# xXCoffeeColaXc/WeatherConverter

Measured on NVIDIA B200. Metric: guided translation images/sec (256x512, T steps) at 1/2/4/8 B200 vs host CPU, higher is better.
Workload: dtype bf16

## Files before the change

include/wc_b200.h:

```cpp
#ifndef WC_B200_H_
#define WC_B200_H_

#include <stddef.h>
#include <stdint.h>

#ifdef __cplusplus
extern "C" {
#endif

typedef uint16_t wc_bf16;

const char* wc_last_error(void);
int wc_abi_version(void);
long long wc_launch_count(void);

void wc_profile_begin(void);
int wc_profile_end(double* ms_by_class, long long* count_by_class, double* work_by_class);
int wc_profile_detail(int cap, int* cls, double* ms, double* work, int* info);

int wc_ddpm_step(const float* xt, const float* eps, const float* z, float* out, float* mean_out, float* sigz_out,
                 size_t n_per_sample, int batch, float beta, float sqrt_one_minus_acp, float sqrt_alpha, float sigma,
                 void* stream);
int wc_ddpm_step_batched(const float* xt, const float* eps, const float* z, float* out, float* mean_out,
                         float* sigz_out, size_t n_per_sample, int batch, const float* betas, const float* alphas,
                         const float* sqrt_one_minus_acp, const int64_t* t, int num_timesteps, void* stream);
int wc_ddpm_step_indexed(const float* xt, const float* eps, const float* z, float* out, float* mean_out, float* sigz_out,
                         size_t n_per_sample, int batch, const float* coef_tables, const int64_t* t_dev, int num_timesteps,
                         void* stream);
int wc_ddim_step(const float* xt, const float* eps, const float* z, float* out, float* mean_out, float* sigz_out,
                 size_t n_per_sample, int batch, float a_t, float s_t, float a_prev, float d, float sigma, void* stream);
int wc_ddim_step_indexed(const float* xt, const float* eps, const float* z, float* out, float* mean_out, float* sigz_out,
                         size_t n_per_sample, int batch, const float* coef_tables, const int64_t* t_dev, int num_timesteps,
                         void* stream);
int wc_add_noise(const float* x0, const float* noise, float* out, size_t n_per_sample, int batch,
                 const float* sqrt_acp, const float* sqrt_one_minus_acp, const int64_t* t, int num_timesteps, void* stream);

int wc_set_time_factor_table(const float* factor_host, int half);
int wc_time_embedding(const int64_t* t, int n, int dim, float* out, void* stream);

int wc_sgg_update(const float* grad, const float* mu, const float* sigz, float* out, float* mag_out, int batch, int h,
                  int w, int pool, float lambda, void* stream);

int wc_lcg_prepare(const float* sr_xt, const int64_t* gt, float* x_masked, int64_t* gt_masked, int batch, int num_classes,
                   int H, int W, void* stream);
int wc_lcg_combine(const float* pooled_grads, const int64_t* gt, const float* mu, const float* sigz, float* out, int batch,
                   int num_classes, int h, int w, int pool, float lambda, void* stream);

size_t wc_groupnorm_workspace_bytes(int batch);
int wc_groupnorm_silu(const wc_bf16* x, wc_bf16* y, int batch, int hw, int channels, int ldx, int ldy,
                      const float* gamma, const float* beta, float eps, int silu, void* workspace, void* stream);
int wc_conv2d(const wc_bf16* x, int batch, int H, int W, int Cin, int ldx, const float* weight, const float* bias,
              int Cout, int K, int stride, int pad, int dil, int transposed, const float* rowbias,
              const wc_bf16* residual, int ldr, const wc_bf16* x2, int Cin2, int ldx2, const float* weight2, int relu,
              wc_bf16* y, int ldy, void* stream);
int wc_conv_in(const float* x, const float* weight, const float* bias, const float* scale, const float* shift,
               wc_bf16* y, int batch, int H, int W, int Cout, int K, int stride, int pad, int ldy, int relu,
               void* stream);
int wc_conv_out(const wc_bf16* x, const float* weight, const float* bias, float* y, int batch, int H, int W, int Cin,
                int K, int ldx, int tanh_out, void* stream);
int wc_conv2d_dgrad(const wc_bf16* dz, int batch, int Ho, int Wo, int Cout, const float* weight, int Cin, int K, int stride,
                    int dil, const wc_bf16* residual, const wc_bf16* mask, wc_bf16* dx, void* stream);
int wc_maxpool3x3s2(const wc_bf16* x, wc_bf16* y, uint8_t* idx, int batch, int H, int W, int C, void* stream);
int wc_maxpool3x3s2_bwd(const wc_bf16* dy, const uint8_t* idx, const wc_bf16* x, wc_bf16* dx, int batch, int H, int W, int C,
                        void* stream);
int wc_bilinear(const wc_bf16* x, wc_bf16* y, int batch, int Hi, int Wi, int Ho, int Wo, int C, void* stream);
int wc_bilinear_bwd(const wc_bf16* dy, const wc_bf16* mask, wc_bf16* dx, int batch, int Hi, int Wi, int Ho, int Wo, int C,
                    void* stream);
int wc_seg_loss_head(const float* logits_lo, const int64_t* labels, int* n_valid_ws, int64_t* pred, float* dlogit_hi,
                     float* loss, float* logits_hi, wc_bf16* dlogit_lo, int batch, int h, int w, int H, int W, void* stream);
int wc_conv1_dgrad(const wc_bf16* dz, const float* weight, const float* scale, float* dx, int batch, int H, int W, void* stream);
int wc_nchw_f32_to_nhwc_bf16(const float* x, wc_bf16* y, int batch, int C, int hw, int ldy, void* stream);
int wc_nhwc_bf16_to_nchw_f32(const wc_bf16* x, float* y, int batch, int C, int hw, int ldx, void* stream);
int wc_attention(const wc_bf16* q, const wc_bf16* k, const wc_bf16* vt, wc_bf16* out, int batch, int heads, int ntok,
                 int hd, int ldo, void* stream);
int wc_attention_scaled(const wc_bf16* q, const wc_bf16* k, const wc_bf16* vt, wc_bf16* out, int batch, int heads, int ntok,
                        int hd, int ldo, float scale, void* stream);

int wc_ddpm_grid_u8(const float* x, uint8_t* out, int batch, int H, int W, int nrow, int padding, void* stream);
int wc_postprocess_u8(const float* x, uint8_t* out, int batch, int H, int W, const float* mean3_host, const float* std3_host, void* stream);
int wc_label_encode(const uint8_t* label_ids, int Ws, const int* ytab, const int* xtab, int top, int left, int Hc, int Wc,
                    const int64_t* lut, int nlut, int64_t* out, void* stream);
int wc_resample_u8(const uint8_t* in, uint8_t* tmp, uint8_t* out, int Hin, int Win, int Hout, int Wout, int channels, const int* bounds_h,
                   const int* kk_h, int ksize_h, const int* bounds_v, const int* kk_v, int ksize_v, void* stream);
int wc_u8_to_tensor(const uint8_t* in, int Win, int top, int left, int Hc, int Wc, int mode, const float* mean3_host, const float* std3_host,
                    float* out, void* stream);

int wc_attention_lse(const wc_bf16* q, const wc_bf16* k, const wc_bf16* vt, wc_bf16* out, float* lse, int batch, int heads,
                     int ntok, int hd, int ldo, void* stream);
int wc_attention_bwd(const wc_bf16* q, const wc_bf16* k, const wc_bf16* v, const wc_bf16* o, const wc_bf16* d_o, const float* lse,
                     float* d_scratch, wc_bf16* dqkv, int batch, int heads, int ntok, int hd, void* stream);
int wc_conv2d_wgrad(const wc_bf16* x, const wc_bf16* dy, int batch, int H, int W, int Cin, int Cout, int K, int stride, int pad,
                    int dil, int transposed, const wc_bf16* x2, int Cin2, float* dw, float* dw2, void* stream);
size_t wc_groupnorm_bwd_workspace_bytes(int batch, int channels);
int wc_groupnorm_silu_bwd(const wc_bf16* x, const wc_bf16* dy, wc_bf16* dx, int batch, int hw, int channels, const float* gamma,
                          const float* beta, float eps, int silu, const void* fwd_workspace, const wc_bf16* add1,
                          const wc_bf16* add2, float* dgamma, float* dbeta, void* workspace, void* stream);
int wc_colsum(const wc_bf16* x, int batch, int hw, int channels, float* out_rows, float* out_total, void* workspace, void* stream);
int wc_mse_loss_grad(const float* pred, const float* target, float* dpred, size_t n, float grad_scale, float* loss, void* scratch,
                     void* stream);
size_t wc_boundary_wgrad_scratch_bytes(void);
int wc_boundary_wgrad(const wc_bf16* wide, const float* narrow, int batch, int H, int W, int sign, float* dw, float* dbias,
                      void* scratch, void* stream);
int wc_adam_step(float* p, const float* g, float* m, float* v, size_t n, float lr, float beta1, float beta2, float eps, int step,
                 float grad_scale, void* stream);

typedef struct wc_unet wc_unet;
typedef struct {
  int im_channels, im_size, time_emb_dim, num_down_layers, num_mid_layers, num_up_layers, num_heads;
  int n_down_channels;
  int down_channels[8];
  int n_mid_channels;
  int mid_channels[8];
  int down_sample[8];
  int n_attn_resolutions;
  int attn_resolutions[8];
} wc_unet_config;
int wc_unet_create(wc_unet** out, const wc_unet_config* cfg, int n_params, const char* const* names,
                   const float* const* ptrs, const int64_t* numels, void* stream);
void wc_unet_destroy(wc_unet* net);
size_t wc_unet_workspace_bytes(const wc_unet* net, int batch, int H, int W);
int wc_unet_forward(wc_unet* net, const float* x, const int64_t* t, int n_t, float* out, int batch, int H, int W,
                    void* workspace, size_t workspace_bytes, void* stream);
double wc_unet_flops(const wc_unet* net);
int wc_unet_launches(const wc_unet* net);

typedef struct wc_unet_train wc_unet_train;
int wc_unet_train_create(wc_unet_train** out, const wc_unet_config* cfg, int n_params, const char* const* names,
                         float* const* params, float* const* grads);
void wc_unet_train_destroy(wc_unet_train* net);
size_t wc_unet_train_workspace_bytes(wc_unet_train* net, int batch, int H, int W);
int wc_unet_train_bind(wc_unet_train* net, int batch, int H, int W, void* workspace, size_t workspace_bytes, void* stream);
int wc_unet_train_forward(wc_unet_train* net, const float* x, const int64_t* t, const float* target, float* pred_out,
                          float* loss_out, float grad_scale, int repack, void* stream);
int wc_unet_train_num_backward_ops(const wc_unet_train* net);
int wc_unet_train_backward(wc_unet_train* net, int op_begin, int op_end, void* stream);
int wc_unet_train_backward_seeded(wc_unet_train* net, const float* dpred, float* dx, int param_grads, void* stream);
int wc_unet_train_grad_ready_op(const wc_unet_train* net, const char* name);
double wc_unet_train_flops(const wc_unet_train* net, int backward);

typedef struct wc_legacy_unet wc_legacy_unet;
int wc_legacy_unet_create(wc_legacy_unet** out, int n_params, const char* const* names, const float* const* ptrs,
                          const int64_t* numels);
void wc_legacy_unet_destroy(wc_legacy_unet* net);
size_t wc_legacy_unet_workspace_bytes(wc_legacy_unet* net, int batch, int size);
int wc_legacy_unet_forward(wc_legacy_unet* net, const float* x, const float* t, float* out, int batch, int size, void* workspace,
                           size_t workspace_bytes, void* stream);
double wc_legacy_unet_flops(const wc_legacy_unet* net);
int wc_legacy_unet_launches(const wc_legacy_unet* net);

typedef struct wc_seg wc_seg;
int wc_seg_create(wc_seg** out, const int* blocks_per_layer, int num_classes, int n_params, const char* const* names,
                  const float* const* ptrs, void* stream);
int wc_seg_set_output_stride(wc_seg* net, int output_stride);
void wc_seg_destroy(wc_seg* net);
size_t wc_seg_workspace_bytes(const wc_seg* net, int batch, int H, int W, int with_grad);
int wc_seg_infer(wc_seg* net, const float* x, const int64_t* labels, int64_t* pred, float* input_grad, float* loss,
                 float* logits, int batch, int H, int W, void* workspace, size_t workspace_bytes, void* stream);
int wc_seg_infer_pooled(wc_seg* net, const float* x, const int64_t* labels, int64_t* pred, float* input_grad, float* loss,
                        float* logits, int batch, int H, int W, int grad_pool, void* workspace, size_t workspace_bytes,
                        void* stream);
int wc_seg_forward(wc_seg* net, const float* x, float* logits, int batch, int H, int W, int save_for_backward, void* workspace,
                   size_t workspace_bytes, void* stream);
int wc_seg_backward_seeded(wc_seg* net, const float* dlogits, float* input_grad, void* stream);
double wc_seg_flops(const wc_seg* net, int backward);
int wc_seg_launches(const wc_seg* net);

typedef struct wc_srgan wc_srgan;
int wc_srgan_create(wc_srgan** out, int num_blocks, int upscale, int n_params, const char* const* names,
                    const float* const* ptrs, void* stream);
void wc_srgan_destroy(wc_srgan* net);
size_t wc_srgan_workspace_bytes(const wc_srgan* net, int batch, int h, int w);
int wc_srgan_forward(wc_srgan* net, const float* x, float* y, int batch, int h, int w, void* workspace,
                     size_t workspace_bytes, void* stream);
size_t wc_srgan_grad_workspace_bytes(const wc_srgan* net, int batch, int h, int w);
int wc_srgan_forward_saved(wc_srgan* net, const float* x, float* y, int batch, int h, int w, void* workspace,
                           size_t workspace_bytes, void* stream);
int wc_srgan_backward_seeded(wc_srgan* net, const float* dy, float* dx, void* stream);
double wc_srgan_flops(const wc_srgan* net);
int wc_srgan_launches(const wc_srgan* net);

#ifdef __cplusplus
}
#endif
#endif
```

weatherconverter_b200/_lib.py:

```python
import ctypes as C
import os

import torch

_HERE = os.path.dirname(os.path.abspath(__file__))
LIB_PATH = os.path.join(_HERE, "libwc_b200.so")

_lib = None

c_f32p = C.c_void_p
c_ptr = C.c_void_p


class UnetConfigStruct(C.Structure):
    _fields_ = [
        ("im_channels", C.c_int), ("im_size", C.c_int), ("time_emb_dim", C.c_int),
        ("num_down_layers", C.c_int), ("num_mid_layers", C.c_int), ("num_up_layers", C.c_int),
        ("num_heads", C.c_int),
        ("n_down_channels", C.c_int), ("down_channels", C.c_int * 8),
        ("n_mid_channels", C.c_int), ("mid_channels", C.c_int * 8),
        ("down_sample", C.c_int * 8),
        ("n_attn_resolutions", C.c_int), ("attn_resolutions", C.c_int * 8),
    ]


_SIGS = {
    "wc_last_error": (C.c_char_p, []),
    "wc_abi_version": (C.c_int, []),
    "wc_launch_count": (C.c_longlong, []),
    "wc_profile_begin": (None, []),
    "wc_profile_detail": (C.c_int, [C.c_int, C.POINTER(C.c_int), C.POINTER(C.c_double), C.POINTER(C.c_double), C.POINTER(C.c_int)]),
    "wc_profile_end": (C.c_int, [C.POINTER(C.c_double), C.POINTER(C.c_longlong), C.POINTER(C.c_double)]),
    "wc_ddpm_step": (C.c_int, [c_ptr] * 6 + [C.c_size_t, C.c_int] + [C.c_float] * 4 + [c_ptr]),
    "wc_ddpm_step_batched": (C.c_int, [c_ptr] * 6 + [C.c_size_t, C.c_int] + [c_ptr] * 4 + [C.c_int, c_ptr]),
    "wc_ddpm_step_indexed": (C.c_int, [c_ptr] * 6 + [C.c_size_t, C.c_int, c_ptr, c_ptr, C.c_int, c_ptr]),
    "wc_ddim_step": (C.c_int, [c_ptr] * 6 + [C.c_size_t, C.c_int] + [C.c_float] * 5 + [c_ptr]),
    "wc_ddim_step_indexed": (C.c_int, [c_ptr] * 6 + [C.c_size_t, C.c_int, c_ptr, c_ptr, C.c_int, c_ptr]),
    "wc_add_noise": (C.c_int, [c_ptr] * 3 + [C.c_size_t, C.c_int] + [c_ptr] * 3 + [C.c_int, c_ptr]),
    "wc_set_time_factor_table": (C.c_int, [C.POINTER(C.c_float), C.c_int]),
    "wc_time_embedding": (C.c_int, [c_ptr, C.c_int, C.c_int, c_ptr, c_ptr]),
    "wc_sgg_update": (C.c_int, [c_ptr] * 5 + [C.c_int] * 4 + [C.c_float, c_ptr]),
    "wc_lcg_prepare": (C.c_int, [c_ptr] * 4 + [C.c_int] * 4 + [c_ptr]),
    "wc_lcg_combine": (C.c_int, [c_ptr] * 5 + [C.c_int] * 5 + [C.c_float, c_ptr]),
    "wc_groupnorm_workspace_bytes": (C.c_size_t, [C.c_int]),
    "wc_groupnorm_silu": (C.c_int, [c_ptr, c_ptr] + [C.c_int] * 5 + [c_ptr, c_ptr, C.c_float, C.c_int, c_ptr, c_ptr]),
    "wc_conv2d": (C.c_int, [c_ptr] + [C.c_int] * 5 + [c_ptr, c_ptr] + [C.c_int] * 6 + [c_ptr, c_ptr, C.c_int, c_ptr,
                            C.c_int, C.c_int, c_ptr, C.c_int, c_ptr, C.c_int, c_ptr]),
    "wc_conv2d_dgrad": (C.c_int, [c_ptr] + [C.c_int] * 4 + [c_ptr] + [C.c_int] * 4 + [c_ptr] * 4),
    "wc_maxpool3x3s2": (C.c_int, [c_ptr] * 3 + [C.c_int] * 4 + [c_ptr]),
    "wc_maxpool3x3s2_bwd": (C.c_int, [c_ptr] * 4 + [C.c_int] * 4 + [c_ptr]),
    "wc_bilinear": (C.c_int, [c_ptr] * 2 + [C.c_int] * 6 + [c_ptr]),
    "wc_bilinear_bwd": (C.c_int, [c_ptr] * 3 + [C.c_int] * 6 + [c_ptr]),
    "wc_seg_loss_head": (C.c_int, [c_ptr] * 8 + [C.c_int] * 5 + [c_ptr]),
    "wc_conv1_dgrad": (C.c_int, [c_ptr] * 4 + [C.c_int] * 3 + [c_ptr]),
    "wc_conv_in": (C.c_int, [c_ptr] * 6 + [C.c_int] * 9 + [c_ptr]),
    "wc_conv_out": (C.c_int, [c_ptr] * 4 + [C.c_int] * 7 + [c_ptr]),
    "wc_nchw_f32_to_nhwc_bf16": (C.c_int, [c_ptr, c_ptr] + [C.c_int] * 4 + [c_ptr]),
    "wc_nhwc_bf16_to_nchw_f32": (C.c_int, [c_ptr, c_ptr] + [C.c_int] * 4 + [c_ptr]),
    "wc_attention": (C.c_int, [c_ptr] * 4 + [C.c_int] * 5 + [c_ptr]),
    "wc_ddpm_grid_u8": (C.c_int, [c_ptr, c_ptr] + [C.c_int] * 5 + [c_ptr]),
    "wc_postprocess_u8": (C.c_int, [c_ptr, c_ptr] + [C.c_int] * 3 + [C.POINTER(C.c_float), C.POINTER(C.c_float), c_ptr]),
    "wc_label_encode": (C.c_int, [c_ptr, C.c_int, c_ptr, c_ptr] + [C.c_int] * 4 + [c_ptr, C.c_int, c_ptr, c_ptr]),
    "wc_resample_u8": (C.c_int, [c_ptr] * 3 + [C.c_int] * 5 + [c_ptr, c_ptr, C.c_int, c_ptr, c_ptr, C.c_int, c_ptr]),
    "wc_u8_to_tensor": (C.c_int, [c_ptr] + [C.c_int] * 6 + [C.POINTER(C.c_float), C.POINTER(C.c_float), c_ptr, c_ptr]),
    "wc_attention_lse": (C.c_int, [c_ptr] * 5 + [C.c_int] * 5 + [c_ptr]),
    "wc_attention_scaled": (C.c_int, [c_ptr] * 4 + [C.c_int] * 5 + [C.c_float, c_ptr]),
    "wc_attention_bwd": (C.c_int, [c_ptr] * 8 + [C.c_int] * 4 + [c_ptr]),
    "wc_conv2d_wgrad": (C.c_int, [c_ptr, c_ptr] + [C.c_int] * 10 + [c_ptr, C.c_int, c_ptr, c_ptr, c_ptr]),
    "wc_groupnorm_bwd_workspace_bytes": (C.c_size_t, [C.c_int, C.c_int]),
    "wc_groupnorm_silu_bwd": (C.c_int, [c_ptr] * 3 + [C.c_int] * 3 + [c_ptr, c_ptr, C.c_float, C.c_int] + [c_ptr] * 7),
    "wc_colsum": (C.c_int, [c_ptr] + [C.c_int] * 3 + [c_ptr] * 4),
    "wc_mse_loss_grad": (C.c_int, [c_ptr] * 3 + [C.c_size_t, C.c_float, c_ptr, c_ptr, c_ptr]),
    "wc_boundary_wgrad_scratch_bytes": (C.c_size_t, []),
    "wc_boundary_wgrad": (C.c_int, [c_ptr, c_ptr] + [C.c_int] * 4 + [c_ptr] * 4),
    "wc_adam_step": (C.c_int, [c_ptr] * 4 + [C.c_size_t] + [C.c_float] * 4 + [C.c_int, C.c_float, c_ptr]),
    "wc_unet_create": (C.c_int, [C.POINTER(c_ptr), C.POINTER(UnetConfigStruct), C.c_int, C.POINTER(C.c_char_p),
                                 C.POINTER(c_ptr), C.POINTER(C.c_int64), c_ptr]),
    "wc_unet_destroy": (None, [c_ptr]),
    "wc_unet_workspace_bytes": (C.c_size_t, [c_ptr, C.c_int, C.c_int, C.c_int]),
    "wc_unet_forward": (C.c_int, [c_ptr, c_ptr, c_ptr, C.c_int, c_ptr, C.c_int, C.c_int, C.c_int, c_ptr, C.c_size_t,
                                  c_ptr]),
    "wc_unet_flops": (C.c_double, [c_ptr]),
    "wc_unet_launches": (C.c_int, [c_ptr]),
    "wc_unet_train_create": (C.c_int, [C.POINTER(c_ptr), C.POINTER(UnetConfigStruct), C.c_int, C.POINTER(C.c_char_p),
                                       C.POINTER(c_ptr), C.POINTER(c_ptr)]),
    "wc_unet_train_destroy": (None, [c_ptr]),
    "wc_unet_train_workspace_bytes": (C.c_size_t, [c_ptr, C.c_int, C.c_int, C.c_int]),
    "wc_unet_train_bind": (C.c_int, [c_ptr, C.c_int, C.c_int, C.c_int, c_ptr, C.c_size_t, c_ptr]),
    "wc_unet_train_forward": (C.c_int, [c_ptr] * 6 + [C.c_float, C.c_int, c_ptr]),
    "wc_unet_train_num_backward_ops": (C.c_int, [c_ptr]),
    "wc_unet_train_backward": (C.c_int, [c_ptr, C.c_int, C.c_int, c_ptr]),
    "wc_unet_train_backward_seeded": (C.c_int, [c_ptr, c_ptr, c_ptr, C.c_int, c_ptr]),
    "wc_unet_train_grad_ready_op": (C.c_int, [c_ptr, C.c_char_p]),
    "wc_unet_train_flops": (C.c_double, [c_ptr, C.c_int]),
    "wc_legacy_unet_create": (C.c_int, [C.POINTER(c_ptr), C.c_int, C.POINTER(C.c_char_p), C.POINTER(c_ptr), C.POINTER(C.c_int64)]),
    "wc_legacy_unet_destroy": (None, [c_ptr]),
    "wc_legacy_unet_workspace_bytes": (C.c_size_t, [c_ptr, C.c_int, C.c_int]),
    "wc_legacy_unet_forward": (C.c_int, [c_ptr, c_ptr, c_ptr, c_ptr, C.c_int, C.c_int, c_ptr, C.c_size_t, c_ptr]),
    "wc_legacy_unet_flops": (C.c_double, [c_ptr]),
    "wc_legacy_unet_launches": (C.c_int, [c_ptr]),
    "wc_seg_create": (C.c_int, [C.POINTER(c_ptr), C.POINTER(C.c_int), C.c_int, C.c_int, C.POINTER(C.c_char_p),
                                C.POINTER(c_ptr), c_ptr]),
    "wc_seg_set_output_stride": (C.c_int, [c_ptr, C.c_int]),
    "wc_seg_destroy": (None, [c_ptr]),
    "wc_seg_workspace_bytes": (C.c_size_t, [c_ptr, C.c_int, C.c_int, C.c_int, C.c_int]),
    "wc_seg_infer": (C.c_int, [c_ptr] * 7 + [C.c_int] * 3 + [c_ptr, C.c_size_t, c_ptr]),
    "wc_seg_infer_pooled": (C.c_int, [c_ptr] * 7 + [C.c_int] * 4 + [c_ptr, C.c_size_t, c_ptr]),
    "wc_seg_forward": (C.c_int, [c_ptr] * 3 + [C.c_int] * 4 + [c_ptr, C.c_size_t, c_ptr]),
    "wc_seg_backward_seeded": (C.c_int, [c_ptr] * 4),
    "wc_seg_flops": (C.c_double, [c_ptr, C.c_int]),
    "wc_seg_launches": (C.c_int, [c_ptr]),
    "wc_srgan_create": (C.c_int, [C.POINTER(c_ptr), C.c_int, C.c_int, C.c_int, C.POINTER(C.c_char_p), C.POINTER(c_ptr), c_ptr]),
    "wc_srgan_destroy": (None, [c_ptr]),
    "wc_srgan_workspace_bytes": (C.c_size_t, [c_ptr, C.c_int, C.c_int, C.c_int]),
    "wc_srgan_forward": (C.c_int, [c_ptr, c_ptr, c_ptr, C.c_int, C.c_int, C.c_int, c_ptr, C.c_size_t, c_ptr]),
    "wc_srgan_grad_workspace_bytes": (C.c_size_t, [c_ptr, C.c_int, C.c_int, C.c_int]),
    "wc_srgan_forward_saved": (C.c_int, [c_ptr, c_ptr, c_ptr, C.c_int, C.c_int, C.c_int, c_ptr, C.c_size_t, c_ptr]),
    "wc_srgan_backward_seeded": (C.c_int, [c_ptr] * 4),
    "wc_srgan_flops": (C.c_double, [c_ptr]),
    "wc_srgan_launches": (C.c_int, [c_ptr]),
}

EXPORTS = tuple(_SIGS.keys())


def lib():
    global _lib
    if _lib is None:
        if not os.path.exists(LIB_PATH):
            raise RuntimeError(
                f"{LIB_PATH} not found: the CUDA extension has not been built "
                "(run __graft_entry__.build()); this package has no CPU fallback")
        handle = C.CDLL(LIB_PATH)
        for name, (res, args) in _SIGS.items():
            fn = getattr(handle, name)
            fn.restype = res
            fn.argtypes = args
        _lib = handle
    return _lib


def check(rc):
    if rc != 0:
        msg = lib().wc_last_error()
        raise RuntimeError("wc_b200: " + (msg.decode() if msg else f"error {rc}"))


def require_cuda(*tensors):
    if not torch.cuda.is_available():
        raise RuntimeError("wc_b200 needs a CUDA device (sm_100a); there is no CPU fallback")
    for t in tensors:
        if t is not None and not t.is_cuda:
            raise RuntimeError("wc_b200 kernels take CUDA tensors; got a tensor on " + str(t.device))


def ptr(t):
    return None if t is None else C.c_void_p(t.data_ptr())


def stream_ptr():
    return C.c_void_p(torch.cuda.current_stream().cuda_stream)
```

weatherconverter_b200/csrc/attention.cu:

```cuda
#include "wc_host.h"
#include "wc_ptx.cuh"

#include <cstdlib>
#include <type_traits>

namespace wc {

namespace {

struct AttnArgs {
  int ntok, heads, ldo;
  float scale_log2;
  __nv_bfloat16* out;
  float* lse;
};

struct AttnMaps {
  CUtensorMap q, k, vt;
};

template <int HD, int BKV, int NQ, bool TP = false>
struct AttnCfg {
  static constexpr int kKBlocks = HD >= 64 ? HD / 64 : 1;
  static constexpr int kSwz = HD >= 64 ? 128 : HD * 2;
  static constexpr int kRowBytes = HD >= 64 ? 128 : HD * 2;
  static constexpr int kKSteps = HD >= 64 ? 4 : HD / 16;
  static constexpr uint32_t kQTile = 128 * HD * 2;
  static constexpr uint32_t kKTile = BKV * HD * 2;
  static constexpr uint32_t kVTile = HD * BKV * 2;
  static constexpr uint32_t kPTile = 128 * BKV * 2;
  static constexpr int kStages = 2;
  static constexpr uint32_t kSmem = NQ * kQTile + kStages * (kKTile + kVTile) + (TP ? 0 : NQ * kPTile) + 1024 + 256;
  static constexpr int kThreads = 128 + 128 * NQ;
  static constexpr int kColsPerQ = BKV + HD + (TP ? BKV / 2 : 0);
  static_assert(NQ * kColsPerQ <= 512, "TMEM budget");
  static constexpr uint32_t kTmemCols = NQ * kColsPerQ <= 256 ? 256 : 512;
};

template <int HD, int BKV, int NQ, int POLY, bool TP>
__global__ void __launch_bounds__(AttnCfg<HD, BKV, NQ, TP>::kThreads, 1)
attention_kernel(const __grid_constant__ AttnMaps maps, const __grid_constant__ AttnArgs p) {
  using Cfg = AttnCfg<HD, BKV, NQ, TP>;
  extern __shared__ uint8_t smem_raw[];
  const uint32_t base = (smem_u32(smem_raw) + 1023u) & ~1023u;
  const uint32_t q_smem = base;
  const uint32_t k_smem = q_smem + NQ * Cfg::kQTile;
  const uint32_t v_smem = k_smem + Cfg::kStages * Cfg::kKTile;
  const uint32_t p_smem = v_smem + Cfg::kStages * Cfg::kVTile;
  const uint32_t bars = p_smem + (TP ? 0u : NQ * Cfg::kPTile);
  const uint32_t q_full = bars;
  auto k_full = [&](int s) { return bars + 8u * (1 + s); };
  auto k_empty = [&](int s) { return bars + 8u * (3 + s); };
  auto v_full = [&](int s) { return bars + 8u * (5 + s); };
  auto v_empty = [&](int s) { return bars + 8u * (7 + s); };
  auto s_full = [&](int q) { return bars + 8u * (9 + q); };
  auto p_full = [&](int q) { return bars + 8u * (12 + q); };
  auto pv_done = [&](int q) { return bars + 8u * (15 + q); };
  const uint32_t tmem_slot = bars + 8u * 18;
  volatile uint32_t* tmem_slot_ptr = reinterpret_cast<volatile uint32_t*>(smem_raw + (tmem_slot - smem_u32(smem_raw)));

  const int warp = __shfl_sync(0xffffffffu, threadIdx.x >> 5, 0), lane = threadIdx.x & 31;
  const int bh = blockIdx.y;
  const int q0 = blockIdx.x * (128 * NQ);
  const int nkv = (p.ntok + BKV - 1) / BKV;

  if (warp == 0 && lane == 0) {
    tma_prefetch_desc(&maps.q);
    tma_prefetch_desc(&maps.k);
    tma_prefetch_desc(&maps.vt);
  }
  if (warp == 1 && lane == 0) {
    mbar_init(q_full, 1);
    for (int s = 0; s < Cfg::kStages; ++s) {
      mbar_init(k_full(s), 1); mbar_init(k_empty(s), 1);
      mbar_init(v_full(s), 1); mbar_init(v_empty(s), 1);
    }
    for (int q = 0; q < NQ; ++q) {
      mbar_init(s_full(q), 1);
      mbar_init(p_full(q), 128);
      mbar_init(pv_done(q), 1);
    }
    fence_barrier_init();
  }
  if (warp == 2) {
    tmem_alloc(tmem_slot, Cfg::kTmemCols);
    tmem_relinquish();
  }
  pdl_launch_dependents();
  pdl_wait();
  tc_fence_before();
  __syncthreads();
  tc_fence_after();
  const uint32_t tmem_base = *tmem_slot_ptr;

  if (warp == 0) {
    if (lane == 0) {
      mbar_arrive_expect_tx(q_full, NQ * Cfg::kQTile);
      for (int q = 0; q < NQ; ++q)
        for (int kb = 0; kb < Cfg::kKBlocks; ++kb)
          tma_load_3d(q_smem + q * Cfg::kQTile + kb * (128 * Cfg::kRowBytes), &maps.q, q_full, kb * 64, q0 + q * 128, bh);
      for (int j = 0; j < nkv; ++j) {
        const int s = j & 1;
        const uint32_t ph = (j >> 1) & 1u;
        mbar_wait(k_empty(s), ph ^ 1u);
        mbar_arrive_expect_tx(k_full(s), Cfg::kKTile);
        for (int kb = 0; kb < Cfg::kKBlocks; ++kb)
          tma_load_3d(k_smem + s * Cfg::kKTile + kb * (BKV * Cfg::kRowBytes), &maps.k, k_full(s), kb * 64, j * BKV, bh);
        mbar_wait(v_empty(s), ph ^ 1u);
        mbar_arrive_expect_tx(v_full(s), Cfg::kVTile);
        for (int vb = 0; vb < BKV / 64; ++vb)
          tma_load_3d(v_smem + s * Cfg::kVTile + vb * (HD * 128), &maps.vt, v_full(s), j * BKV + vb * 64, 0, bh);
      }
    }
  } else if (warp == 1) {
    {
      const uint32_t tmem_base = __shfl_sync(0xffffffffu, *tmem_slot_ptr, 0);
      const uint32_t idesc_s = umma_idesc_bf16(128, BKV);
      const uint32_t idesc_o = umma_idesc_bf16(128, HD);
      const uint64_t dq = umma_smem_desc(q_smem, Cfg::kSwz, 8 * Cfg::kRowBytes);
      const uint64_t dp = umma_smem_desc(p_smem, 128, 1024);
      const uint32_t hi_qk = umma_desc_hi(dq), hi_pv = umma_desc_hi(dp);
      const uint32_t q_lo0 = umma_desc_lo(dq), k_lo0 = q_lo0 + ((k_smem - q_smem) >> 4);
      const uint32_t p_lo0 = umma_desc_lo(dp), v_lo0 = p_lo0 - ((p_smem - v_smem) >> 4);
      auto issue_s = [&](int q, int j) {
        const uint32_t d = tmem_base + q * Cfg::kColsPerQ;
        const uint32_t q_lo = q_lo0 + q * (Cfg::kQTile >> 4), k_lo = k_lo0 + (j & 1) * (Cfg::kKTile >> 4);
#pragma unroll
        for (int kb = 0; kb < Cfg::kKBlocks; ++kb) {
#pragma unroll
          for (int k = 0; k < Cfg::kKSteps; ++k)
            umma_bf16(d, umma_desc_join(q_lo + kb * ((128 * Cfg::kRowBytes) >> 4) + 2u * k, hi_qk),
                      umma_desc_join(k_lo + kb * ((BKV * Cfg::kRowBytes) >> 4) + 2u * k, hi_qk), idesc_s, (kb | k) != 0 ? 1u : 0u);
        }
        umma_commit(s_full(q));
      };
      auto issue_pv = [&](int q, int j) {
        const uint32_t d = tmem_base + q * Cfg::kColsPerQ + BKV;
        const uint32_t p_lo = p_lo0 + q * (Cfg::kPTile >> 4), v_lo = v_lo0 + (j & 1) * (Cfg::kVTile >> 4);
#pragma unroll
        for (int vb = 0; vb < BKV / 64; ++vb) {
#pragma unroll
          for (int k = 0; k < 4; ++k)
            if (TP)
              umma_bf16_ts(d, d + HD + 8u * (vb * 4 + k), umma_desc_join(v_lo + vb * ((HD * 128) >> 4) + 2u * k, hi_pv), idesc_o,
                           (j | vb | k) != 0 ? 1u : 0u);
            else
              umma_bf16(d, umma_desc_join(p_lo + vb * ((128 * 128) >> 4) + 2u * k, hi_pv),
                        umma_desc_join(v_lo + vb * ((HD * 128) >> 4) + 2u * k, hi_pv), idesc_o, (j | vb | k) != 0 ? 1u : 0u);
        }
        umma_commit(pv_done(q));
      };
      mbar_wait(q_full, 0);
      mbar_wait(k_full(0), 0);
      tc_fence_after();
      if (elect_one_sync()) {
        for (int q = 0; q < NQ; ++q) issue_s(q, 0);
        umma_commit(k_empty(0));
      }
      __syncwarp();
      for (int j = 0; j < nkv; ++j) {
        const int s = j & 1;
        const uint32_t ph = (j >> 1) & 1u;
        mbar_wait(v_full(s), ph);
        const bool more = (j + 1 < nkv);
        if (more) mbar_wait(k_full((j + 1) & 1), ((j + 1) >> 1) & 1u);
#pragma unroll
        for (int q = 0; q < NQ; ++q) {
          mbar_wait(p_full(q), j & 1u);
          tc_fence_after();
          if (elect_one_sync()) {
            issue_pv(q, j);
            if (more) issue_s(q, j + 1);
          }
          __syncwarp();
        }
        if (elect_one_sync()) {
          umma_commit(v_empty(s));
          if (more) umma_commit(k_empty((j + 1) & 1));
        }
        __syncwarp();
      }
    }
  } else if (warp >= 4) {
    const int q = (warp - 4) >> 2;
    const int quad = warp & 3;
    const int row = quad * 32 + lane;
    const uint32_t lane_off = static_cast<uint32_t>(quad * 32) << 16;
    const uint32_t s_tmem = tmem_base + q * Cfg::kColsPerQ + lane_off;
    const uint32_t o_tmem = s_tmem + BKV;
    const uint32_t p_row = p_smem + q * Cfg::kPTile + row * 128;
    const float sl2 = p.scale_log2;
    float m = -INFINITY;
    float2 lsum[2] = {make_float2(0.f, 0.f), make_float2(0.f, 0.f)};
    auto tile = [&](int j, auto tail_tag) {
      constexpr bool TAIL = decltype(tail_tag)::value;
      const int kv0 = j * BKV;
      constexpr int NCH = BKV / 32;
      uint32_t ra[32], rb[32];
      float tm[8];
#pragma unroll
      for (int i = 0; i < 8; ++i) tm[i] = -INFINITY;
      tmem_ld32(s_tmem, ra);
#pragma unroll
      for (int c = 0; c < NCH; ++c) {
        tmem_wait_ld();
        uint32_t(&cur)[32] = (c & 1) ? rb : ra;
        if (c + 1 < NCH) tmem_ld32(s_tmem + 32 * (c + 1), (c & 1) ? ra : rb);
#pragma unroll
        for (int i = 0; i < 32; i += 2) {
          float a = __uint_as_float(cur[i]), b2 = __uint_as_float(cur[i + 1]);
          if (TAIL) {
            if (kv0 + 32 * c + i >= p.ntok) a = -INFINITY;
            if (kv0 + 32 * c + i + 1 >= p.ntok) b2 = -INFINITY;
          }
          tm[(i >> 1) & 7] = fmaxf(tm[(i >> 1) & 7], fmaxf(a, b2));
        }
      }
      const float tmax = fmaxf(fmaxf(fmaxf(tm[0], tm[1]), fmaxf(tm[2], tm[3])), fmaxf(fmaxf(tm[4], tm[5]), fmaxf(tm[6], tm[7])));
      tmem_ld32(s_tmem, ra);
      if (j > 0) mbar_wait(pv_done(q), (j - 1) & 1u);
      tc_fence_after();
      if (j == 0) {
        m = tmax;
      } else {
        const bool grow = (tmax - m) * sl2 > 8.0f;
        if (__any_sync(0xffffffffu, grow)) {
          const float m_new = fmaxf(m, tmax);
          const float alpha = ex2_approx((m - m_new) * sl2);
#pragma unroll
          for (int i = 0; i < 2; ++i) { lsum[i].x *= alpha; lsum[i].y *= alpha; }
          m = m_new;
          tmem_wait_ld();
#pragma unroll
          for (int c0 = 0; c0 < HD; c0 += 16) {
            uint32_t r[16];
            tmem_ld16(o_tmem + c0, r);
            tmem_wait_ld();
#pragma unroll
            for (int i = 0; i < 16; ++i) r[i] = __float_as_uint(__uint_as_float(r[i]) * alpha);
            tmem_st16(o_tmem + c0, r);
          }
          tmem_wait_st();
        }
      }
      const float mneg = -m * sl2;
#pragma unroll
      for (int c = 0; c < NCH; ++c) {
        tmem_wait_ld();
        uint32_t(&cur)[32] = (c & 1) ? rb : ra;
        if (c + 1 < NCH) tmem_ld32(s_tmem + 32 * (c + 1), (c & 1) ? ra : rb);
        float pv[32];
        const float2 sl2v = make_float2(sl2, sl2), mnegv = make_float2(mneg, mneg);
#pragma unroll
        for (int i = 0; i < 32; i += 2) {
          const float2 xs = ffma2(make_float2(__uint_as_float(cur[i]), __uint_as_float(cur[i + 1])), sl2v, mnegv);
          float2 v;
          if (i < POLY) {
            v = exp2_poly2(xs);
          } else {
            v.x = ex2_approx(xs.x);
            v.y = ex2_approx(xs.y);
          }
          if (TAIL) {
            if (kv0 + 32 * c + i >= p.ntok) v.x = 0.f;
            if (kv0 + 32 * c + i + 1 >= p.ntok) v.y = 0.f;
          }
          pv[i] = v.x; pv[i + 1] = v.y;
          lsum[(i >> 1) & 1] = fadd2(lsum[(i >> 1) & 1], v);
        }
        if (TP) {
          uint32_t w[16];
#pragma unroll
          for (int i = 0; i < 16; ++i) w[i] = pack_bf16(pv[2 * i], pv[2 * i + 1]);
          tmem_st16(o_tmem + HD + 16 * c, w);
          continue;
        }
        const uint32_t blk = p_row + ((32 * c) >> 6) * (128 * 128);
#pragma unroll
        for (int ch = 0; ch < 4; ++ch) {
          const int chunk = (((32 * c) & 63) >> 3) + ch;
          const uint32_t addr = blk + (static_cast<uint32_t>(chunk ^ (row & 7)) << 4);
          const uint32_t w0 = pack_bf16(pv[8 * ch + 0], pv[8 * ch + 1]), w1 = pack_bf16(pv[8 * ch + 2], pv[8 * ch + 3]);
          const uint32_t w2 = pack_bf16(pv[8 * ch + 4], pv[8 * ch + 5]), w3 = pack_bf16(pv[8 * ch + 6], pv[8 * ch + 7]);
          asm volatile("st.shared.v4.b32 [%0], {%1,%2,%3,%4};" ::"r"(addr), "r"(w0), "r"(w1), "r"(w2), "r"(w3) : "memory");
        }
      }
      if (TP) tmem_wait_st();
      else fence_proxy_async_smem();
      tc_fence_before();
      mbar_arrive(p_full(q));
    };
    for (int j = 0; j < nkv; ++j) {
      mbar_wait(s_full(q), j & 1u);
      tc_fence_after();
      if (j * BKV + BKV > p.ntok) tile(j, std::true_type{});
      else tile(j, std::false_type{});
    }
    const float l = (lsum[0].x + lsum[0].y) + (lsum[1].x + lsum[1].y);
    mbar_wait(pv_done(q), (nkv - 1) & 1u);
    tc_fence_after();
    const int tok = q0 + q * 128 + row;
    const float inv = 1.f / l;
    const int b = bh / p.heads, head = bh % p.heads;
    if (p.lse && tok < p.ntok) p.lse[static_cast<size_t>(bh) * p.ntok + tok] = fmaf(m, sl2, log2f(l));
    __nv_bfloat16* dst = p.out + (static_cast<size_t>(b) * p.ntok + tok) * p.ldo + head * HD;
#pragma unroll
    for (int c0 = 0; c0 < HD; c0 += 16) {
      uint32_t r[16];
      tmem_ld16(o_tmem + c0, r);
      tmem_wait_ld();
      if (tok < p.ntok) {
        uint4 u0, u1;
        u0.x = pack_bf16(__uint_as_float(r[0]) * inv, __uint_as_float(r[1]) * inv);
        u0.y = pack_bf16(__uint_as_float(r[2]) * inv, __uint_as_float(r[3]) * inv);
        u0.z = pack_bf16(__uint_as_float(r[4]) * inv, __uint_as_float(r[5]) * inv);
        u0.w = pack_bf16(__uint_as_float(r[6]) * inv, __uint_as_float(r[7]) * inv);
        u1.x = pack_bf16(__uint_as_float(r[8]) * inv, __uint_as_float(r[9]) * inv);
        u1.y = pack_bf16(__uint_as_float(r[10]) * inv, __uint_as_float(r[11]) * inv);
        u1.z = pack_bf16(__uint_as_float(r[12]) * inv, __uint_as_float(r[13]) * inv);
        u1.w = pack_bf16(__uint_as_float(r[14]) * inv, __uint_as_float(r[15]) * inv);
        *reinterpret_cast<uint4*>(dst + c0) = u0;
        *reinterpret_cast<uint4*>(dst + c0 + 8) = u1;
      }
    }
  }
  tc_fence_before();
  __syncthreads();
  if (warp == 2) {
    tc_fence_after();
    tmem_dealloc(tmem_base, Cfg::kTmemCols);
  }
}

template <int HD, int BKV, int NQ, int POLY, bool TP>
int launch_attention_p(const __nv_bfloat16* q, const __nv_bfloat16* k, const __nv_bfloat16* vt, __nv_bfloat16* out, int B,
                     int heads, int ntok, int ldo, cudaStream_t st, float* lse, float scale) {
  using Cfg = AttnCfg<HD, BKV, NQ, TP>;
  AttnMaps maps;
  const int BH = B * heads;
  const uint32_t inner = HD >= 64 ? 64 : HD;
  {
    uint64_t dims[3] = {static_cast<uint64_t>(HD), static_cast<uint64_t>(ntok), static_cast<uint64_t>(BH)};
    uint64_t strides[3] = {1, static_cast<uint64_t>(HD), static_cast<uint64_t>(HD) * ntok};
    uint32_t boxq[3] = {inner, 128, 1};
    uint32_t boxk[3] = {inner, static_cast<uint32_t>(BKV), 1};
    if (int e = encode_tmap_bf16(&maps.q, q, 3, dims, strides, boxq, Cfg::kSwz)) return e;
    if (int e = encode_tmap_bf16(&maps.k, k, 3, dims, strides, boxk, Cfg::kSwz)) return e;
  }
  {
    uint64_t dims[3] = {static_cast<uint64_t>(ntok), static_cast<uint64_t>(HD), static_cast<uint64_t>(BH)};
    uint64_t strides[3] = {1, static_cast<uint64_t>(ntok), static_cast<uint64_t>(HD) * ntok};
    uint32_t box[3] = {64, static_cast<uint32_t>(HD), 1};
    if (int e = encode_tmap_bf16(&maps.vt, vt, 3, dims, strides, box, 128)) return e;
  }
  AttnArgs args;
  args.ntok = ntok; args.heads = heads; args.ldo = ldo; args.out = out; args.lse = lse;
  args.scale_log2 = attn_scale_log2(scale, HD);
  static bool attr_set = false;
  if (!attr_set) {
    WC_CHECK_CUDA(cudaFuncSetAttribute(attention_kernel<HD, BKV, NQ, POLY, TP>, cudaFuncAttributeMaxDynamicSharedMemorySize,
                                       Cfg::kSmem));
    attr_set = true;
  }
  dim3 grid((ntok + 128 * NQ - 1) / (128 * NQ), BH);
  ProfScope prof(kProfAttention, st, 4.0 * BH * static_cast<double>(ntok) * ntok * HD);
  prof.note(BH, ntok, HD);
  launch_k<1>(attention_kernel<HD, BKV, NQ, POLY, TP>, grid, Cfg::kThreads, Cfg::kSmem, st, maps, args);
  WC_LAUNCH_CHECK();
  return 0;
}

template <int HD, int BKV, int NQ, bool TP = false>
int launch_attention(const __nv_bfloat16* q, const __nv_bfloat16* k, const __nv_bfloat16* vt, __nv_bfloat16* out, int B,
                     int heads, int ntok, int ldo, cudaStream_t st, float* lse, float scale) {
  static int poly = -1;
  if (poly < 0) {
    const char* e = getenv("WC_ATTN_POLY");
    poly = e ? atoi(e) : 14;
  }
  switch (poly) {
    case 0: return launch_attention_p<HD, BKV, NQ, 0, TP>(q, k, vt, out, B, heads, ntok, ldo, st, lse, scale);
    case 8: return launch_attention_p<HD, BKV, NQ, 8, TP>(q, k, vt, out, B, heads, ntok, ldo, st, lse, scale);
    case 20: return launch_attention_p<HD, BKV, NQ, 20, TP>(q, k, vt, out, B, heads, ntok, ldo, st, lse, scale);
    default: return launch_attention_p<HD, BKV, NQ, 14, TP>(q, k, vt, out, B, heads, ntok, ldo, st, lse, scale);
  }
}

}

int attention_small_forward(const __nv_bfloat16* q, const __nv_bfloat16* k, const __nv_bfloat16* vt, __nv_bfloat16* out, int B,
                            int heads, int ntok, int hd, int ldo, cudaStream_t st, float* lse, float scale);
int attention_small4_forward(const __nv_bfloat16* q, const __nv_bfloat16* k, const __nv_bfloat16* vt, __nv_bfloat16* out, int B,
                             int heads, int ntok, int hd, int ldo, cudaStream_t st, float* lse, float scale);

int attention_forward(const __nv_bfloat16* q, const __nv_bfloat16* k, const __nv_bfloat16* vt, __nv_bfloat16* out, int B,
                      int heads, int ntok, int hd, int ldo, cudaStream_t st, float* lse, float scale) {
  WC_REQUIRE(ntok % 8 == 0, "token count must be a multiple of 8");
  WC_REQUIRE(ldo % 8 == 0, "output row stride must be a multiple of 8");
  static int small = -1;
  if (small < 0) {
    const char* e = getenv("WC_ATTN_SMALL");
    small = e ? atoi(e) : 1;
  }
  if (small && (hd == 16 || hd == 32)) {
    static int four = -1;
    if (four < 0) {
      const char* e = getenv("WC_ATTN_SMALL4");
      four = e ? atoi(e) : 1;
    }
    static int four32 = -1;
    if (four32 < 0) {
      const char* e = getenv("WC_ATTN_SMALL4_HD32");
      four32 = e ? atoi(e) : 1;
    }
    if (four && (hd == 16 || (hd == 32 && four32)) && ntok >= 2048) return attention_small4_forward(q, k, vt, out, B, heads, ntok, hd, ldo, st, lse, scale);
    return attention_small_forward(q, k, vt, out, B, heads, ntok, hd, ldo, st, lse, scale);
  }
  static int tp = -1;
  if (tp < 0) {
    const char* e = getenv("WC_ATTN_TP");
    tp = e ? atoi(e) : 1;
  }
  if (tp) {
    switch (hd) {
      case 64: return launch_attention<64, 128, 2, true>(q, k, vt, out, B, heads, ntok, ldo, st, lse, scale);
      case 128: return launch_attention<128, 64, 2, true>(q, k, vt, out, B, heads, ntok, ldo, st, lse, scale);
      case 192: return launch_attention<192, 64, 1, true>(q, k, vt, out, B, heads, ntok, ldo, st, lse, scale);
      default: break;
    }
  }
  switch (hd) {
    case 16: return launch_attention<16, 128, 3>(q, k, vt, out, B, heads, ntok, ldo, st, lse, scale);
    case 32: return launch_attention<32, 128, 3>(q, k, vt, out, B, heads, ntok, ldo, st, lse, scale);
    case 64: return launch_attention<64, 128, 2>(q, k, vt, out, B, heads, ntok, ldo, st, lse, scale);
    case 128: return launch_attention<128, 64, 2>(q, k, vt, out, B, heads, ntok, ldo, st, lse, scale);
    case 192: return launch_attention<192, 64, 1>(q, k, vt, out, B, heads, ntok, ldo, st, lse, scale);
    default: return fail("attention: unsupported head_dim " + std::to_string(hd) + " (supported: 16,32,64,128,192)");
  }
}

double attention_flops(int B, int heads, int ntok, int hd) { return 4.0 * B * heads * static_cast<double>(ntok) * ntok * hd; }

}
```

weatherconverter_b200/csrc/attention_small4.cu:

```cuda
#include "wc_host.h"
#include "wc_ptx.cuh"

#include <cstdlib>
#include <type_traits>

namespace wc {

namespace {

struct Small4Args {
  int ntok, heads, ldo;
  float qscale;
  float c;
  __nv_bfloat16* out;
  float* lse;
};

struct Small4Maps {
  CUtensorMap q, k, vt;
};

constexpr int kBKV = 64;
constexpr int kNQ = 4;
constexpr int kKStages = 4;
constexpr float kShift = 8.0f;
constexpr float kLazy = 6.0f;
#ifndef WC_S4_SERVICE_REGS
#define WC_S4_SERVICE_REGS 56
#define WC_S4_SOFTMAX_REGS 104
#endif
constexpr int kRegsService = WC_S4_SERVICE_REGS, kRegsSoftmax = WC_S4_SOFTMAX_REGS;
static_assert(128 * kRegsService + 512 * kRegsSoftmax <= 640 * 96, "register pool of the CTA");

template <int HD>
struct Cfg4 {
  static constexpr bool kLT = true;
  static constexpr int kRowBytes = HD * 2;
  static constexpr int kSwz = HD * 2;
  static constexpr int kKSteps = HD / 16;
  static constexpr int kVRows = HD + (kLT ? 16 : 0);
  static constexpr uint32_t kQTile = 128 * HD * 2;
  static constexpr uint32_t kXTile = 128 * 32;
  static constexpr uint32_t kKxTile = kBKV * 32;
  static constexpr uint32_t kKTile = kBKV * HD * 2;
  static constexpr uint32_t kVBlock = kVRows * 128;
  static constexpr uint32_t kVLoad = HD * 128;
  static constexpr uint32_t kPTile = 128 * kBKV * 2;
  static constexpr uint32_t kSmem = kNQ * kQTile + kNQ * kXTile + kKxTile + kKStages * (kKTile + kVBlock) + 2 * kNQ * kPTile + 1024 + 512;
  static constexpr int kThreads = 128 + 128 * kNQ;
  static constexpr int kColsPerQ = kBKV + kVRows;
  static_assert(kNQ * kColsPerQ <= 512, "TMEM budget");
  static constexpr uint32_t kTmemCols = 512;
};

__device__ __forceinline__ void sts128(uint32_t addr, uint32_t a, uint32_t b, uint32_t c, uint32_t d) {
  asm volatile("st.shared.v4.b32 [%0], {%1,%2,%3,%4};" ::"r"(addr), "r"(a), "r"(b), "r"(c), "r"(d) : "memory");
}
__device__ __forceinline__ void lds128(uint32_t addr, uint32_t (&v)[4]) {
  asm volatile("ld.shared.v4.b32 {%0,%1,%2,%3}, [%4];" : "=r"(v[0]), "=r"(v[1]), "=r"(v[2]), "=r"(v[3]) : "r"(addr) : "memory");
}
__device__ __forceinline__ void sts16(uint32_t addr, uint16_t v) {
  asm volatile("st.shared.u16 [%0], %1;" ::"r"(addr), "h"(v) : "memory");
}
__device__ __forceinline__ float bf16_round(float x) { return __bfloat162float(__float2bfloat16_rn(x)); }
__device__ __forceinline__ uint16_t bf16_bits(float x) {
  __nv_bfloat16 h = __float2bfloat16_rn(x);
  return *reinterpret_cast<uint16_t*>(&h);
}
__device__ __forceinline__ float2 fmul2(float2 a, float2 b) {
  unsigned long long ua = *reinterpret_cast<unsigned long long*>(&a), ub = *reinterpret_cast<unsigned long long*>(&b), ud;
  asm("mul.rn.f32x2 %0, %1, %2;" : "=l"(ud) : "l"(ua), "l"(ub));
  return *reinterpret_cast<float2*>(&ud);
}
__device__ __forceinline__ float2 exp2_poly2_scaled(float2 x, float2 c, float lo) {
  const float kMagic = 12582912.f;
  x.x = fmaxf(x.x, lo);
  x.y = fmaxf(x.y, lo);
  const float2 r = ffma2(x, c, make_float2(kMagic, kMagic));
  const float2 nn = ffma2(r, make_float2(-1.f, -1.f), make_float2(kMagic, kMagic));
  const float2 f = ffma2(x, c, nn);
  float2 p = ffma2(f, make_float2(0.05517163872718811f, 0.05517163872718811f), make_float2(0.2426111251115799f, 0.2426111251115799f));
  p = ffma2(p, f, make_float2(0.6932609677314758f, 0.6932609677314758f));
  p = ffma2(p, f, make_float2(0.9999280571937561f, 0.9999280571937561f));
  float2 o;
  o.x = __uint_as_float((__float_as_uint(r.x) << 23) + __float_as_uint(p.x));
  o.y = __uint_as_float((__float_as_uint(r.y) << 23) + __float_as_uint(p.y));
  return o;
}

template <int HD, int POLY, bool UNIT>
__global__ void __launch_bounds__(Cfg4<HD>::kThreads, 1)
attention_small4_kernel(const __grid_constant__ Small4Maps maps, const __grid_constant__ Small4Args p) {
  using Cfg = Cfg4<HD>;
  constexpr bool LT = Cfg::kLT;
  extern __shared__ uint8_t smem_raw[];
  const uint32_t base = (smem_u32(smem_raw) + 1023u) & ~1023u;
  const uint32_t q_smem = base;
  const uint32_t qx_smem = q_smem + kNQ * Cfg::kQTile;
  const uint32_t kx_smem = qx_smem + kNQ * Cfg::kXTile;
  const uint32_t k_smem = kx_smem + Cfg::kKxTile;
  const uint32_t v_smem = k_smem + kKStages * Cfg::kKTile;
  const uint32_t p_smem = v_smem + kKStages * Cfg::kVBlock;
  const uint32_t bars = p_smem + 2 * kNQ * Cfg::kPTile;
  const uint32_t q_full = bars;
  auto k_full = [&](int s) { return bars + 8u * (1 + s); };
  auto k_empty = [&](int s) { return bars + 8u * (5 + s); };
  auto v_full = [&](int s) { return bars + 8u * (9 + s); };
  auto v_empty = [&](int s) { return bars + 8u * (13 + s); };
  auto s_full = [&](int q) { return bars + 8u * (17 + q); };
  auto s_free = [&](int q) { return bars + 8u * (21 + q); };
  auto p_full = [&](int q, int b) { return bars + 8u * (25 + 2 * q + b); };
  auto pv_done = [&](int q, int b) { return bars + 8u * (33 + 2 * q + b); };
  auto q_ready = [&](int q) { return bars + 8u * (41 + q); };
  const uint32_t tmem_slot = bars + 8u * 45;
  volatile uint32_t* tmem_slot_ptr = reinterpret_cast<volatile uint32_t*>(smem_raw + (tmem_slot - smem_u32(smem_raw)));

  const int warp = __shfl_sync(0xffffffffu, threadIdx.x >> 5, 0), lane = threadIdx.x & 31;
  const int bh = HD == 16 ? blockIdx.x : blockIdx.y;
  const int q0 = (HD == 16 ? blockIdx.y : blockIdx.x) * (128 * kNQ);
  const int nkv = (p.ntok + kBKV - 1) / kBKV;
  const int nq_valid = min(kNQ, (p.ntok - q0 + 127) / 128);

  if (warp == 0 && lane == 0) {
    tma_prefetch_desc(&maps.q);
    tma_prefetch_desc(&maps.k);
    tma_prefetch_desc(&maps.vt);
  }
  if (warp == 1 && lane == 0) {
    mbar_init(q_full, 1);
    for (int s = 0; s < kKStages; ++s) {
      mbar_init(k_full(s), 1); mbar_init(k_empty(s), 1);
      mbar_init(v_full(s), 1); mbar_init(v_empty(s), 1);
    }
    for (int q = 0; q < kNQ; ++q) {
      mbar_init(s_full(q), 1);
      mbar_init(s_free(q), 128);
      for (int b = 0; b < 2; ++b) {
        mbar_init(p_full(q, b), 128);
        mbar_init(pv_done(q, b), 1);
      }
      mbar_init(q_ready(q), 128);
    }
    fence_barrier_init();
  }
  if (warp == 2) {
    tmem_alloc(tmem_slot, Cfg::kTmemCols);
    tmem_relinquish();
  }
  pdl_launch_dependents();
  pdl_wait();
  tc_fence_before();
  __syncthreads();
  tc_fence_after();
  const uint32_t tmem_base = *tmem_slot_ptr;

  if (warp < 4) {
    asm volatile("setmaxnreg.dec.sync.aligned.u32 %0;" ::"n"(kRegsService));
    if (warp == 0) {
      if (lane == 0) {
        mbar_arrive_expect_tx(q_full, kNQ * Cfg::kQTile);
        for (int q = 0; q < kNQ; ++q) tma_load_3d(q_smem + q * Cfg::kQTile, &maps.q, q_full, 0, q0 + q * 128, bh);
        for (int j = 0; j < nkv; ++j) {
          const int s = j % kKStages;
          const uint32_t ph = (j / kKStages) & 1u;
          mbar_wait(k_empty(s), ph ^ 1u);
          mbar_arrive_expect_tx(k_full(s), Cfg::kKTile);
          tma_load_3d(k_smem + s * Cfg::kKTile, &maps.k, k_full(s), 0, j * kBKV, bh);
          mbar_wait(v_empty(s), ph ^ 1u);
          mbar_arrive_expect_tx(v_full(s), Cfg::kVLoad);
          tma_load_3d(v_smem + s * Cfg::kVBlock, &maps.vt, v_full(s), j * kBKV, 0, bh);
        }
      }
    } else if (warp == 1) {
      const uint32_t tmem_u = __shfl_sync(0xffffffffu, tmem_base, 0);
      const uint32_t idesc_s = umma_idesc_bf16(128, kBKV);
      const uint64_t dq = umma_smem_desc(q_smem, Cfg::kSwz, 8 * Cfg::kRowBytes);
      const uint64_t dx = umma_smem_desc(qx_smem, 32, 256);
      const uint32_t hi_qk = umma_desc_hi(dq), hi_x = umma_desc_hi(dx);
      const uint32_t q_lo0 = umma_desc_lo(dq), k_lo0 = q_lo0 + ((k_smem - q_smem) >> 4);
      const uint32_t qx_lo0 = umma_desc_lo(dx), kx_lo = qx_lo0 + ((kx_smem - qx_smem) >> 4);
      auto issue_s = [&](int q, int j) {
        const uint32_t d = tmem_u + q * Cfg::kColsPerQ;
        const uint32_t q_lo = q_lo0 + q * (Cfg::kQTile >> 4), k_lo = k_lo0 + (j % kKStages) * (Cfg::kKTile >> 4);
#pragma unroll
        for (int k = 0; k < Cfg::kKSteps; ++k)
          umma_bf16(d, umma_desc_join(q_lo + 2u * k, hi_qk), umma_desc_join(k_lo + 2u * k, hi_qk), idesc_s, k != 0 ? 1u : 0u);
        umma_bf16(d, umma_desc_join(qx_lo0 + q * (Cfg::kXTile >> 4), hi_x), umma_desc_join(kx_lo, hi_x), idesc_s, 1u);
        umma_commit(s_full(q));
      };
      mbar_wait(k_full(0), 0);
#pragma unroll
      for (int q = 0; q < kNQ; ++q) {
        mbar_wait(q_ready(q), 0);
        tc_fence_after();
        if (q < nq_valid) {
          if (elect_one_sync()) issue_s(q, 0);
          __syncwarp();
        }
      }
      if (elect_one_sync()) umma_commit(k_empty(0));
      __syncwarp();
      for (int j = 0; j + 1 < nkv; ++j) {
        const int s1 = (j + 1) % kKStages;
        mbar_wait(k_full(s1), ((j + 1) / kKStages) & 1u);
#pragma unroll
        for (int q = 0; q < kNQ; ++q) {
          if (q < nq_valid) {
            mbar_wait(s_free(q), j & 1u);
            tc_fence_after();
            if (elect_one_sync()) issue_s(q, j + 1);
            __syncwarp();
          }
        }
        if (elect_one_sync()) umma_commit(k_empty(s1));
        __syncwarp();
      }
    } else if (warp == 3) {
      const uint32_t tmem_u = __shfl_sync(0xffffffffu, tmem_base, 0);
      const uint32_t idesc_o = umma_idesc_bf16(128, Cfg::kVRows);
      const uint64_t dp = umma_smem_desc(p_smem, 128, 1024);
      const uint32_t hi_pv = umma_desc_hi(dp);
      const uint32_t p_lo0 = umma_desc_lo(dp), v_lo0 = p_lo0 - ((p_smem - v_smem) >> 4);
      for (int j = 0; j < nkv; ++j) {
        const int s = j % kKStages;
        mbar_wait(v_full(s), (j / kKStages) & 1u);
#pragma unroll
        for (int q = 0; q < kNQ; ++q) {
          if (q < nq_valid) {
            mbar_wait(p_full(q, j & 1), (j >> 1) & 1u);
            tc_fence_after();
            if (elect_one_sync()) {
              const uint32_t d = tmem_u + q * Cfg::kColsPerQ + kBKV;
              const uint32_t p_lo = p_lo0 + (2 * q + (j & 1)) * (Cfg::kPTile >> 4), v_lo = v_lo0 + s * (Cfg::kVBlock >> 4);
#pragma unroll
              for (int k = 0; k < 4; ++k)
                umma_bf16(d, umma_desc_join(p_lo + 2u * k, hi_pv), umma_desc_join(v_lo + 2u * k, hi_pv), idesc_o, (j | k) != 0 ? 1u : 0u);
              umma_commit(pv_done(q, j & 1));
            }
            __syncwarp();
          }
        }
        if (elect_one_sync()) umma_commit(v_empty(s));
        __syncwarp();
      }
    }
  } else {
    asm volatile("setmaxnreg.inc.sync.aligned.u32 %0;" ::"n"(kRegsSoftmax));
    const int q = (warp - 4) >> 2;
    const int quad = warp & 3;
    const int row = quad * 32 + lane;
    const uint32_t lane_off = static_cast<uint32_t>(quad * 32) << 16;
    const uint32_t s_tmem = tmem_base + q * Cfg::kColsPerQ + lane_off;
    const uint32_t o_tmem = s_tmem + kBKV;
    const uint32_t p_row = p_smem + 2 * q * Cfg::kPTile + row * 128;
    const uint32_t qx_row = qx_smem + q * Cfg::kXTile + row * 32;

    const float cs = p.c;
    const float shift = kShift / cs;
    float E = bf16_round(shift);
    {
      const int t = threadIdx.x - 128;
      if (q == 0 && row < kBKV) {
        sts128(kx_smem + row * 32, 0x00003F80u, 0u, 0u, 0u);
        sts128(kx_smem + row * 32 + 16, 0x00003F80u, 0u, 0u, 0u);
      }
      if (LT) {
        constexpr int kChunks = kKStages * 16 * 8;
        for (int c = t; c < kChunks; c += 128 * kNQ) {
          const int blk = c >> 7, r = (c >> 3) & 15, ch = c & 7;
          const uint32_t one = r == 0 ? 0x3F803F80u : 0u;
          sts128(v_smem + blk * Cfg::kVBlock + (HD + r) * 128 + ch * 16, one, one, one, one);
        }
      }
      mbar_wait(q_full, 0);
      const uint32_t q_row = q_smem + q * Cfg::kQTile + row * Cfg::kRowBytes;
      const float qs = p.qscale;
#pragma unroll
      for (int c = 0; c < (UNIT ? 0 : Cfg::kRowBytes / 16); ++c) {
        uint32_t v[4];
        lds128(q_row + 16 * c, v);
#pragma unroll
        for (int i = 0; i < 4; ++i) {
          const float2 f = unpack_bf16(v[i]);
          v[i] = pack_bf16(f.x * qs, f.y * qs);
        }
        sts128(q_row + 16 * c, v[0], v[1], v[2], v[3]);
      }
      sts128(qx_row, static_cast<uint32_t>(bf16_bits(-E)), 0u, 0u, 0u);
      sts128(qx_row + 16, 0u, 0u, 0u, 0u);
      fence_proxy_async_smem();
      mbar_arrive(q_ready(q));
    }

    float2 lsum[2] = {make_float2(0.f, 0.f), make_float2(0.f, 0.f)};
    float carry = 0.f;

    for (int j = 0; j < (q < nq_valid ? nkv : 0); ++j) {
      const int b = j & 1;
      const int kv0 = j * kBKV;
      mbar_wait(s_full(q), j & 1u);
      if (j >= 2) mbar_wait(pv_done(q, b), ((j - 2) >> 1) & 1u);
      tc_fence_after();
      uint32_t ra[32], rb[32], w[16];
      tmem_ld32(s_tmem, ra);
      tmem_ld32(s_tmem + 32, rb);
      tmem_wait_ld();
      tc_fence_before();
      mbar_arrive(s_free(q));
      const bool tail = (kv0 + kBKV > p.ntok);
      bool slow = tail || j == 0 || __any_sync(0xffffffffu, carry != 0.f);
      const uint32_t blk = p_row + b * Cfg::kPTile;
      if (!slow) {
        uint32_t orw = 0u;
        float2 ts[2] = {make_float2(0.f, 0.f), make_float2(0.f, 0.f)};
        const float2 cv = make_float2(cs, cs);
        const float lo = -125.f / cs;
        auto half = [&](const uint32_t (&cur)[32], int c) {
#pragma unroll
          for (int i = 0; i < 32; i += 2) {
            const float2 xs = make_float2(__uint_as_float(cur[i]), __uint_as_float(cur[i + 1]));
            float2 v;
            if (i < POLY) {
              v = exp2_poly2_scaled(xs, cv, lo);
            } else {
              const float2 y = UNIT ? xs : fmul2(xs, cv);
              v.x = ex2_approx(y.x);
              v.y = ex2_approx(y.y);
            }
            if (!LT) ts[(i >> 1) & 1] = fadd2(ts[(i >> 1) & 1], v);
            w[i >> 1] = pack_bf16(v.x, v.y);
          }
          if (LT) {
#pragma unroll
            for (int i = 0; i < 16; i += 2) orw |= w[i] | w[i + 1];
          }
#pragma unroll
          for (int ch = 0; ch < 4; ++ch) {
            const int chunk = 4 * c + ch;
            sts128(blk + (static_cast<uint32_t>(chunk ^ (row & 7)) << 4), w[4 * ch], w[4 * ch + 1], w[4 * ch + 2], w[4 * ch + 3]);
          }
        };
        half(ra, 0);
        half(rb, 1);
        bool redo;
        if (LT) {
          redo = (orw & 0xC000C000u) != 0u;
        } else {
          const float tsum = (ts[0].x + ts[0].y) + (ts[1].x + ts[1].y);
          redo = !(tsum < 32.f);
        }
        slow = __any_sync(0xffffffffu, redo);
        if (!LT && !slow) { lsum[0] = fadd2(lsum[0], ts[0]); lsum[1] = fadd2(lsum[1], ts[1]); }
      }
      if (slow) {
        float tmax = -INFINITY;
#pragma unroll
        for (int i = 0; i < 32; ++i) {
          float a0 = __uint_as_float(ra[i]), a1 = __uint_as_float(rb[i]);
          if (tail && kv0 + i >= p.ntok) a0 = -INFINITY;
          if (tail && kv0 + 32 + i >= p.ntok) a1 = -INFINITY;
          tmax = fmaxf(tmax, fmaxf(a0, a1));
        }
        tmax -= carry;
        float delta = 0.f;
        const bool upd = (j == 0) || (tmax > -shift + kLazy / cs);
        if (upd) {
          if (j + 1 < nkv) mbar_wait(s_full(q), (j + 1) & 1u);
          const float e_new = bf16_round(E + tmax + shift);
          delta = e_new - E;
          E = e_new;
          sts16(qx_row, bf16_bits(-e_new));
        }
        if (j > 0 && __any_sync(0xffffffffu, upd)) {
          mbar_wait(pv_done(q, (j - 1) & 1), ((j - 1) >> 1) & 1u);
          tc_fence_after();
          const float alpha = ex2_approx(-delta * cs);
          if (!LT) {
#pragma unroll
            for (int i = 0; i < 2; ++i) { lsum[i].x *= alpha; lsum[i].y *= alpha; }
          }
#pragma unroll
          for (int c0 = 0; c0 < Cfg::kVRows; c0 += 16) {
            uint32_t r[16];
            tmem_ld16(o_tmem + c0, r);
            tmem_wait_ld();
#pragma unroll
            for (int i = 0; i < 16; ++i) r[i] = __float_as_uint(__uint_as_float(r[i]) * alpha);
            tmem_st16(o_tmem + c0, r);
          }
          tmem_wait_st();
        }
        const float dneg = -(carry + delta) * cs;
        carry = delta;
        auto redo_half = [&](const uint32_t (&cur)[32], int c, float2& acc) {
          const int k0 = kv0 + 32 * c;
#pragma unroll
          for (int i = 0; i < 32; i += 2) {
            float v0 = ex2_approx(fmaf(__uint_as_float(cur[i]), cs, dneg)), v1 = ex2_approx(fmaf(__uint_as_float(cur[i + 1]), cs, dneg));
            if (tail) {
              if (k0 + i >= p.ntok) v0 = 0.f;
              if (k0 + i + 1 >= p.ntok) v1 = 0.f;
            }
            if (!LT) { acc.x += v0; acc.y += v1; }
            w[i >> 1] = pack_bf16(v0, v1);
          }
#pragma unroll
          for (int ch = 0; ch < 4; ++ch) {
            const int chunk = 4 * c + ch;
            sts128(blk + (static_cast<uint32_t>(chunk ^ (row & 7)) << 4), w[4 * ch], w[4 * ch + 1], w[4 * ch + 2], w[4 * ch + 3]);
          }
        };
        redo_half(ra, 0, lsum[0]);
        redo_half(rb, 1, lsum[1]);
      }
      fence_proxy_async_smem();
      tc_fence_before();
      mbar_arrive(p_full(q, b));
    }

    if (q < nq_valid) mbar_wait(pv_done(q, (nkv - 1) & 1), ((nkv - 1) >> 1) & 1u);
    tc_fence_after();
    const int tok = q0 + q * 128 + row;
    const int bb = bh / p.heads, head = bh % p.heads;
    __nv_bfloat16* dst = p.out + (static_cast<size_t>(bb) * p.ntok + tok) * p.ldo + head * HD;
    uint32_t r[Cfg::kVRows];
#pragma unroll
    for (int c0 = 0; c0 < Cfg::kVRows; c0 += 16) {
      uint32_t t16[16];
      tmem_ld16(o_tmem + c0, t16);
      tmem_wait_ld();
#pragma unroll
      for (int i = 0; i < 16; ++i) r[c0 + i] = t16[i];
    }
    const float l = LT ? __uint_as_float(r[HD]) : (lsum[0].x + lsum[0].y) + (lsum[1].x + lsum[1].y);
    const float inv = 1.f / l;
    if (tok < p.ntok) {
      if (p.lse) p.lse[static_cast<size_t>(bh) * p.ntok + tok] = fmaf(cs, E, log2f(l));
#pragma unroll
      for (int c0 = 0; c0 < HD; c0 += 8) {
        uint4 u;
        u.x = pack_bf16(__uint_as_float(r[c0 + 0]) * inv, __uint_as_float(r[c0 + 1]) * inv);
        u.y = pack_bf16(__uint_as_float(r[c0 + 2]) * inv, __uint_as_float(r[c0 + 3]) * inv);
        u.z = pack_bf16(__uint_as_float(r[c0 + 4]) * inv, __uint_as_float(r[c0 + 5]) * inv);
        u.w = pack_bf16(__uint_as_float(r[c0 + 6]) * inv, __uint_as_float(r[c0 + 7]) * inv);
        *reinterpret_cast<uint4*>(dst + c0) = u;
      }
    }
  }
  tc_fence_before();
  __syncthreads();
  if (warp == 2) {
    tc_fence_after();
    tmem_dealloc(tmem_base, Cfg::kTmemCols);
  }
}

template <int HD, int POLY, bool UNIT>
int launch_small4_p(const __nv_bfloat16* q, const __nv_bfloat16* k, const __nv_bfloat16* vt, __nv_bfloat16* out, int B, int heads,
                    int ntok, int ldo, cudaStream_t st, float* lse, float scale) {
  using Cfg = Cfg4<HD>;
  Small4Maps maps;
  const int BH = B * heads;
  {
    uint64_t dims[3] = {static_cast<uint64_t>(HD), static_cast<uint64_t>(ntok), static_cast<uint64_t>(BH)};
    uint64_t strides[3] = {1, static_cast<uint64_t>(HD), static_cast<uint64_t>(HD) * ntok};
    uint32_t boxq[3] = {static_cast<uint32_t>(HD), 128, 1};
    uint32_t boxk[3] = {static_cast<uint32_t>(HD), static_cast<uint32_t>(kBKV), 1};
    if (int e = encode_tmap_bf16(&maps.q, q, 3, dims, strides, boxq, Cfg::kSwz)) return e;
    if (int e = encode_tmap_bf16(&maps.k, k, 3, dims, strides, boxk, Cfg::kSwz)) return e;
  }
  {
    uint64_t dims[3] = {static_cast<uint64_t>(ntok), static_cast<uint64_t>(HD), static_cast<uint64_t>(BH)};
    uint64_t strides[3] = {1, static_cast<uint64_t>(ntok), static_cast<uint64_t>(HD) * ntok};
    uint32_t box[3] = {64, static_cast<uint32_t>(HD), 1};
    if (int e = encode_tmap_bf16(&maps.vt, vt, 3, dims, strides, box, 128)) return e;
  }
  Small4Args args;
  args.ntok = ntok; args.heads = heads; args.ldo = ldo; args.out = out; args.lse = lse;
  {
    const float sl2 = attn_scale_log2(scale, HD);
    int ex = 0;
    const float mant = frexpf(sl2, &ex);
    args.c = mant * 2.f;
    args.qscale = ldexpf(1.f, ex - 1);
  }
  static bool attr_set = false;
  if (!attr_set) {
    WC_CHECK_CUDA(cudaFuncSetAttribute(attention_small4_kernel<HD, POLY, UNIT>, cudaFuncAttributeMaxDynamicSharedMemorySize, Cfg::kSmem));
    attr_set = true;
  }
  const int nqb = (ntok + 128 * kNQ - 1) / (128 * kNQ);
  dim3 grid(HD == 16 ? BH : nqb, HD == 16 ? nqb : BH);
  ProfScope prof(kProfAttention, st, 4.0 * BH * static_cast<double>(ntok) * ntok * HD);
  prof.note(BH, ntok, HD);
  launch_k<1>(attention_small4_kernel<HD, POLY, UNIT>, grid, Cfg::kThreads, Cfg::kSmem, st, maps, args);
  WC_LAUNCH_CHECK();
  return 0;
}

template <int HD>
int launch_small4(const __nv_bfloat16* q, const __nv_bfloat16* k, const __nv_bfloat16* vt, __nv_bfloat16* out, int B, int heads,
                  int ntok, int ldo, cudaStream_t st, float* lse, float scale) {
  static int poly = -1;
  if (poly < 0) {
    const char* e = getenv("WC_ATTN_SMALL4_POLY");
    poly = e ? atoi(e) : 8;
  }
  const bool unit = attn_scale_log2(scale, HD) == 1.f;
  {
    if (unit) {
      switch (poly) {
        case 8: return launch_small4_p<HD, 8, true>(q, k, vt, out, B, heads, ntok, ldo, st, lse, scale);
        case 16: return launch_small4_p<HD, 16, true>(q, k, vt, out, B, heads, ntok, ldo, st, lse, scale);
        default: return launch_small4_p<HD, 12, true>(q, k, vt, out, B, heads, ntok, ldo, st, lse, scale);
      }
    }
  }
  switch (poly) {
    case 8: return launch_small4_p<HD, 8, false>(q, k, vt, out, B, heads, ntok, ldo, st, lse, scale);
    case 16: return launch_small4_p<HD, 16, false>(q, k, vt, out, B, heads, ntok, ldo, st, lse, scale);
    default: return launch_small4_p<HD, 12, false>(q, k, vt, out, B, heads, ntok, ldo, st, lse, scale);
  }
}

}

int attention_small4_forward(const __nv_bfloat16* q, const __nv_bfloat16* k, const __nv_bfloat16* vt, __nv_bfloat16* out, int B,
                             int heads, int ntok, int hd, int ldo, cudaStream_t st, float* lse, float scale) {
  switch (hd) {
    case 16: return launch_small4<16>(q, k, vt, out, B, heads, ntok, ldo, st, lse, scale);
    case 32: return launch_small4<32>(q, k, vt, out, B, heads, ntok, ldo, st, lse, scale);
    default: return fail("attention_small4: unsupported head_dim " + std::to_string(hd));
  }
}

}
```

weatherconverter_b200/csrc/wc_api.cu:

```cuda
#include "../../include/wc_b200.h"

#include "conv.cuh"
#include "wgrad.cuh"

namespace wc {
int ddpm_step(const float* xt, const float* eps, const float* z, float* out, float* mean_out, float* sigz_out,
              size_t n_per_sample, int B, float beta, float s, float sqrt_alpha, float sigma, cudaStream_t st);
int ddpm_step_batched(const float* xt, const float* eps, const float* z, float* out, float* mean_out, float* sigz_out,
                      size_t n_per_sample, int B, const float* betas, const float* alphas, const float* sqrt_1m_acp,
                      const long long* t, int T, cudaStream_t st);
int ddpm_step_indexed(const float* xt, const float* eps, const float* z, float* out, float* mean_out, float* sigz_out,
                      size_t n_per_sample, int B, const float* coef_tables, const long long* t_dev, int T, cudaStream_t st);
int ddim_step(const float* xt, const float* eps, const float* z, float* out, float* mean_out, float* sigz_out,
              size_t n_per_sample, int B, float a_t, float s_t, float a_prev, float d, float sigma, cudaStream_t st);
int ddim_step_indexed(const float* xt, const float* eps, const float* z, float* out, float* mean_out, float* sigz_out,
                      size_t n_per_sample, int B, const float* coef_tables, const long long* t_dev, int T, cudaStream_t st);
int add_noise(const float* x0, const float* noise, float* out, size_t n_per_sample, int B, const float* sqrt_acp,
              const float* sqrt_1m_acp, const long long* t, int T, cudaStream_t st);
int sgg_update(const float* grad, const float* mu, const float* sigz, float* out, float* mag_out, int B, int h, int w,
               int pool, float lam, cudaStream_t st);
int lcg_prepare(const float* sr, const long long* gt, float* xm, long long* gm, int B, int NC, size_t hw, cudaStream_t st);
int lcg_combine(const float* g4, const long long* gt, const float* mu, const float* sigz, float* out, int B, int NC, int h,
                int w, int pool, float lam, cudaStream_t st);
int groupnorm_silu(const __nv_bfloat16* x, __nv_bfloat16* y, int B, int HW, int C, int ld, int ldy, const float* gamma,
                   const float* beta, float eps, int silu, void* workspace, cudaStream_t st);
size_t groupnorm_workspace_bytes(int B);
int conv_small_cin(const float* x, const float* w, const float* bias, const float* scale, const float* shift,
                   __nv_bfloat16* y, int B, int Cin, int H, int W, int Cout, int K, int stride, int pad, int ldy,
                   int relu, cudaStream_t st, const float* prelu = nullptr);
int conv_small_cout(const __nv_bfloat16* x, const float* w, const float* bias, float* y, int B, int H, int W, int Cin,
                    int Cout, int K, int ldx, int tanh_out, cudaStream_t st);
int nchw_f32_to_nhwc_bf16(const float* x, __nv_bfloat16* y, int B, int C, int HW, int ldy, cudaStream_t st);
int nhwc_bf16_to_nchw_f32(const __nv_bfloat16* x, float* y, int B, int C, int HW, int ldx, cudaStream_t st);
void prof_start();
int prof_detail(int cap, int* cls, double* ms, double* work, int* info);
int prof_stop(double* ms, long long* count, double* work);
int attention_forward(const __nv_bfloat16* q, const __nv_bfloat16* k, const __nv_bfloat16* vt, __nv_bfloat16* out, int B,
                      int heads, int ntok, int hd, int ldo, cudaStream_t st, float* lse = nullptr, float scale = 0.f);
int maxpool_fwd(const __nv_bfloat16* x, __nv_bfloat16* y, uint8_t* idx, int B, int H, int W, int C, cudaStream_t st);
int maxpool_bwd(const __nv_bfloat16* dy, const uint8_t* idx, const __nv_bfloat16* x, __nv_bfloat16* dx, int B, int H,
                int W, int C, cudaStream_t st);
int bilinear_fwd(const __nv_bfloat16* x, __nv_bfloat16* y, int B, int Hi, int Wi, int Ho, int Wo, int C, int ldx, int ldy,
                 cudaStream_t st);
int bilinear_bwd(const __nv_bfloat16* dy, const __nv_bfloat16* mask, __nv_bfloat16* dx, int B, int Hi, int Wi, int Ho,
                 int Wo, int C, int ldy, int ldm, int ldx, cudaStream_t st);
int seg_loss_grad(const float* logits_lo, const long long* labels, int* n_valid, long long* pred, float* dlogit_hi,
                  float* loss, float* logits_hi, int B, int h, int w, int H, int W, int nc, int ignore, cudaStream_t st);
int seg_loss_head_fused(const float* logits_lo, const long long* labels, int* n_valid, long long* pred, float* loss,
                        __nv_bfloat16* dlo, int B, int h, int w, int H, int W, int nc, int cp, int ldo, int ignore, cudaStream_t st);
int logits_bilinear_bwd(const float* dhi, __nv_bfloat16* dlo, int B, int h, int w, int H, int W, int nc, int cp, int ldo,
                        cudaStream_t st);
int conv1_dgrad(const __nv_bfloat16* dz, const float* w, const float* scale, float* dx, int B, int H, int W, int Cout,
                cudaStream_t st);
int groupnorm_silu_bwd(const __nv_bfloat16* x, const __nv_bfloat16* dy, __nv_bfloat16* dx, int B, int HW, int C, int ld,
                       int ldd, int ldo, const float* gamma, const float* beta, float eps, int silu, const void* stats,
                       const __nv_bfloat16* add1, int lda1, const __nv_bfloat16* add2, int lda2, float* dgamma, float* dbeta,
                       void* workspace, cudaStream_t st);
size_t groupnorm_bwd_workspace_bytes(int B, int Cmax);
int colsum(const __nv_bfloat16* x, int B, int HW, int C, int ld, float* out_rows, int ldo, float* out_total, void* workspace,
           cudaStream_t st);
int attention_backward(const __nv_bfloat16* q, const __nv_bfloat16* k, const __nv_bfloat16* v, const __nv_bfloat16* d_o, int ldd,
                       const float* lse, const float* D, __nv_bfloat16* dqkv, int ld3, int B, int heads, int ntok, int hd,
                       cudaStream_t st);
int attn_rowdot(const __nv_bfloat16* o, const __nv_bfloat16* d_o, int ldo, int ldd, int B, int ntok, int heads, int hd, float* D,
                cudaStream_t st);
int mse_loss_grad(const float* pred, const float* target, float* dpred, size_t n, float grad_scale, float* loss, void* scratch,
                  cudaStream_t st);
size_t boundary_wgrad_scratch_bytes();
int boundary_wgrad(const __nv_bfloat16* wide, int ldw, const float* narrow, int B, int H, int W, int sign, float* dw,
                   float* dbias, void* scratch, cudaStream_t st);
int adam_step(float* p, const float* g, float* m, float* v, size_t n, float lr, float beta1, float beta2, float eps, int step,
              float grad_scale, cudaStream_t st);
int time_embedding(const long long* t, int n, int dim, float* out, cudaStream_t st);
int ddpm_grid_u8(const float* x, uint8_t* out, int B, int H, int W, int nrow, int pad, cudaStream_t st);
int postprocess_u8(const float* x, uint8_t* out, int B, int H, int W, const float* mean3, const float* std3, cudaStream_t st);
int label_encode(const uint8_t* lab, int Ws, const int* ytab, const int* xtab, int top, int left, int Hc, int Wc, const long long* lut,
                 int nlut, long long* out, cudaStream_t st);
int resample_u8(const uint8_t* in, uint8_t* tmp, uint8_t* out, int Hin, int Win, int Hout, int Wout, int C, const int* bounds_h,
                const int* kk_h, int ksize_h, const int* bounds_v, const int* kk_v, int ksize_v, cudaStream_t st);
int u8_to_tensor(const uint8_t* in, int Win, int top, int left, int Hc, int Wc, int mode, const float* mean3, const float* std3, float* out,
                 cudaStream_t st);
}

using namespace wc;
static inline cudaStream_t S(void* s) { return static_cast<cudaStream_t>(s); }
static inline __nv_bfloat16* BF(wc_bf16* p) { return reinterpret_cast<__nv_bfloat16*>(p); }
static inline const __nv_bfloat16* BF(const wc_bf16* p) { return reinterpret_cast<const __nv_bfloat16*>(p); }

extern "C" {

const char* wc_last_error(void) { return last_error_cstr(); }
int wc_abi_version(void) { return 6; }
long long wc_launch_count(void) { return launch_count(); }
void wc_profile_begin(void) { prof_start(); }
int wc_profile_detail(int cap, int* cls, double* ms, double* work, int* info) { return prof_detail(cap, cls, ms, work, info); }
int wc_profile_end(double* ms_by_class, long long* count_by_class, double* work_by_class) {
  return prof_stop(ms_by_class, count_by_class, work_by_class);
}

int wc_ddpm_step(const float* xt, const float* eps, const float* z, float* out, float* mean_out, float* sigz_out,
                 size_t n_per_sample, int batch, float beta, float sqrt_one_minus_acp, float sqrt_alpha, float sigma,
                 void* stream) {
  return ddpm_step(xt, eps, z, out, mean_out, sigz_out, n_per_sample, batch, beta, sqrt_one_minus_acp, sqrt_alpha, sigma,
                   S(stream));
}
int wc_ddpm_step_batched(const float* xt, const float* eps, const float* z, float* out, float* mean_out,
                         float* sigz_out, size_t n_per_sample, int batch, const float* betas, const float* alphas,
                         const float* sqrt_one_minus_acp, const int64_t* t, int num_timesteps, void* stream) {
  return ddpm_step_batched(xt, eps, z, out, mean_out, sigz_out, n_per_sample, batch, betas, alphas, sqrt_one_minus_acp,
                           reinterpret_cast<const long long*>(t), num_timesteps, S(stream));
}
int wc_ddpm_step_indexed(const float* xt, const float* eps, const float* z, float* out, float* mean_out, float* sigz_out,
                         size_t n_per_sample, int batch, const float* coef_tables, const int64_t* t_dev, int num_timesteps,
                         void* stream) {
  return ddpm_step_indexed(xt, eps, z, out, mean_out, sigz_out, n_per_sample, batch, coef_tables,
                           reinterpret_cast<const long long*>(t_dev), num_timesteps, S(stream));
}
int wc_ddim_step(const float* xt, const float* eps, const float* z, float* out, float* mean_out, float* sigz_out,
                 size_t n_per_sample, int batch, float a_t, float s_t, float a_prev, float d, float sigma, void* stream) {
  return ddim_step(xt, eps, z, out, mean_out, sigz_out, n_per_sample, batch, a_t, s_t, a_prev, d, sigma, S(stream));
}
int wc_ddim_step_indexed(const float* xt, const float* eps, const float* z, float* out, float* mean_out, float* sigz_out,
                         size_t n_per_sample, int batch, const float* coef_tables, const int64_t* t_dev, int num_timesteps,
                         void* stream) {
  return ddim_step_indexed(xt, eps, z, out, mean_out, sigz_out, n_per_sample, batch, coef_tables,
                           reinterpret_cast<const long long*>(t_dev), num_timesteps, S(stream));
}
int wc_add_noise(const float* x0, const float* noise, float* out, size_t n_per_sample, int batch,
                 const float* sqrt_acp, const float* sqrt_one_minus_acp, const int64_t* t, int num_timesteps, void* stream) {
  return add_noise(x0, noise, out, n_per_sample, batch, sqrt_acp, sqrt_one_minus_acp,
                   reinterpret_cast<const long long*>(t), num_timesteps, S(stream));
}
int wc_set_time_factor_table(const float* factor_host, int half) { return set_time_factor_table(factor_host, half); }
int wc_time_embedding(const int64_t* t, int n, int dim, float* out, void* stream) {
  return time_embedding(reinterpret_cast<const long long*>(t), n, dim, out, S(stream));
}
int wc_sgg_update(const float* grad, const float* mu, const float* sigz, float* out, float* mag_out, int batch, int h,
                  int w, int pool, float lambda, void* stream) {
  return sgg_update(grad, mu, sigz, out, mag_out, batch, h, w, pool, lambda, S(stream));
}
int wc_lcg_prepare(const float* sr_xt, const int64_t* gt, float* x_masked, int64_t* gt_masked, int batch, int num_classes,
                   int H, int W, void* stream) {
  return lcg_prepare(sr_xt, reinterpret_cast<const long long*>(gt), x_masked, reinterpret_cast<long long*>(gt_masked), batch,
                     num_classes, static_cast<size_t>(H) * W, S(stream));
}
int wc_lcg_combine(const float* pooled_grads, const int64_t* gt, const float* mu, const float* sigz, float* out, int batch,
                   int num_classes, int h, int w, int pool, float lambda, void* stream) {
  return lcg_combine(pooled_grads, reinterpret_cast<const long long*>(gt), mu, sigz, out, batch, num_classes, h, w, pool, lambda,
                     S(stream));
}
size_t wc_groupnorm_workspace_bytes(int batch) { return groupnorm_workspace_bytes(batch); }
int wc_groupnorm_silu(const wc_bf16* x, wc_bf16* y, int batch, int hw, int channels, int ldx, int ldy,
                      const float* gamma, const float* beta, float eps, int silu, void* workspace, void* stream) {
  return groupnorm_silu(BF(x), BF(y), batch, hw, channels, ldx, ldy, gamma, beta, eps, silu, workspace, S(stream));
}

int wc_conv2d(const wc_bf16* x, int batch, int H, int W, int Cin, int ldx, const float* weight, const float* bias,
              int Cout, int K, int stride, int pad, int dil, int transposed, const float* rowbias,
              const wc_bf16* residual, int ldr, const wc_bf16* x2, int Cin2, int ldx2, const float* weight2, int relu,
              wc_bf16* y, int ldy, void* stream) {
  cudaStream_t st = S(stream);
  DeviceArena arena;
  ConvOp op;
  Act xin; xin.ptr = const_cast<__nv_bfloat16*>(BF(x)); xin.B = batch; xin.H = H; xin.W = W; xin.C = Cin; xin.ld = ldx;
  const int Ho = transposed ? H * 2 : (stride == 2 ? H / 2 : H), Wo = transposed ? W * 2 : (stride == 2 ? W / 2 : W);
  Act yout; yout.ptr = BF(y); yout.B = batch; yout.H = Ho; yout.W = Wo; yout.C = Cout; yout.ld = ldy;
  Act res; res.ptr = const_cast<__nv_bfloat16*>(BF(residual)); res.B = batch; res.H = Ho; res.W = Wo; res.C = Cout; res.ld = ldr;
  Act x2a; x2a.ptr = const_cast<__nv_bfloat16*>(BF(x2)); x2a.B = batch; x2a.H = H; x2a.W = W; x2a.C = Cin2; x2a.ld = ldx2;
  Epilogue ep; ep.bias = bias; ep.rowbias = rowbias; ep.ldrb = Cout; ep.res = residual ? &res : nullptr; ep.relu = relu;
  OutSpec os; os.mode = kOutNHWC; os.out = yout;
  int e;
  if (transposed) {
    WC_REQUIRE(stride == 2, "transposed convolution supports stride 2");
    WeightSrc w; w.w = weight; w.d0 = Cin; w.d1 = Cout; w.KH = w.KW = K; w.transpose = 1;
    e = build_conv_transposed_s2(&op, &arena, xin, w, K, pad, Cout, ep, os, st);
  } else {
    WeightSrc w; w.w = weight; w.d0 = Cout; w.d1 = Cin; w.KH = w.KW = K;
    WeightSrc w2; w2.w = weight2; w2.d0 = Cout; w2.d1 = Cin2;
    ConvGeom g; g.K = K; g.stride = stride; g.pad = pad; g.dil = dil;
    e = build_conv(&op, &arena, xin, w, g, Cout, x2 ? &x2a : nullptr, x2 ? &w2 : nullptr, ep, os, st);
  }
  if (e) return e;
  if ((e = op.run(st))) return e;
  WC_CHECK_CUDA(cudaStreamSynchronize(st));
  return 0;
}

int wc_conv2d_dgrad(const wc_bf16* dz, int batch, int Ho, int Wo, int Cout, const float* weight, int Cin, int K, int stride,
                    int dil, const wc_bf16* residual, const wc_bf16* mask, wc_bf16* dx, void* stream) {
  cudaStream_t st = S(stream);
  DeviceArena arena;
  ConvOp op;
  const int H = Ho * stride, W = Wo * stride;
  Act g; g.ptr = const_cast<__nv_bfloat16*>(BF(dz)); g.B = batch; g.H = Ho; g.W = Wo; g.C = Cout; g.ld = Cout;
  Act out; out.ptr = BF(dx); out.B = batch; out.H = H; out.W = W; out.C = Cin; out.ld = Cin;
  Act res = out; res.ptr = const_cast<__nv_bfloat16*>(BF(residual));
  Act msk = out; msk.ptr = const_cast<__nv_bfloat16*>(BF(mask));
  WeightSrc w; w.w = weight; w.d0 = Cout; w.d1 = Cin; w.KH = w.KW = K; w.transpose = 1;
  Epilogue ep; ep.res = residual ? &res : nullptr; ep.mask = mask ? &msk : nullptr;
  OutSpec os; os.mode = kOutNHWC; os.out = out;
  int e;
  if (stride == 1) {
    w.flip = 1;
    ConvGeom gg; gg.K = K; gg.stride = 1; gg.dil = dil; gg.pad = dil * (K - 1) / 2;
    e = build_conv(&op, &arena, g, w, gg, Cin, nullptr, nullptr, ep, os, st);
  } else {
    if (!residual) WC_CHECK_CUDA(cudaMemsetAsync(out.ptr, 0, out.pixels() * Cin * 2, st));
    e = build_conv_transposed_s2(&op, &arena, g, w, K, K == 3 ? 1 : 0, Cin, ep, os, st);
  }
  if (e) return e;
  if ((e = op.run(st))) return e;
  WC_CHECK_CUDA(cudaStreamSynchronize(st));
  return 0;
}
int wc_maxpool3x3s2(const wc_bf16* x, wc_bf16* y, uint8_t* idx, int batch, int H, int W, int C, void* stream) {
  return maxpool_fwd(BF(x), BF(y), idx, batch, H, W, C, S(stream));
}
int wc_maxpool3x3s2_bwd(const wc_bf16* dy, const uint8_t* idx, const wc_bf16* x, wc_bf16* dx, int batch, int H, int W, int C,
                        void* stream) {
  return maxpool_bwd(BF(dy), idx, BF(x), BF(dx), batch, H, W, C, S(stream));
}
int wc_bilinear(const wc_bf16* x, wc_bf16* y, int batch, int Hi, int Wi, int Ho, int Wo, int C, void* stream) {
  return bilinear_fwd(BF(x), BF(y), batch, Hi, Wi, Ho, Wo, C, C, C, S(stream));
}
int wc_bilinear_bwd(const wc_bf16* dy, const wc_bf16* mask, wc_bf16* dx, int batch, int Hi, int Wi, int Ho, int Wo, int C,
                    void* stream) {
  return bilinear_bwd(BF(dy), BF(mask), BF(dx), batch, Hi, Wi, Ho, Wo, C, C, C, C, S(stream));
}
int wc_seg_loss_head(const float* logits_lo, const int64_t* labels, int* n_valid_ws, int64_t* pred, float* dlogit_hi,
                     float* loss, float* logits_hi, wc_bf16* dlogit_lo, int batch, int h, int w, int H, int W, void* stream) {
  if (!dlogit_hi) {
    WC_REQUIRE(dlogit_lo && !logits_hi, "wc_seg_loss_head without dlogit_hi needs dlogit_lo and no logits_hi");
    const int e = seg_loss_head_fused(logits_lo, reinterpret_cast<const long long*>(labels), n_valid_ws, reinterpret_cast<long long*>(pred), loss,
                                      BF(dlogit_lo), batch, h, w, H, W, 19, 32, 32, 255, S(stream));
    if (e == -1) return fail("wc_seg_loss_head: the fused path needs integer up-sampling factors; pass dlogit_hi for the two-pass path");
    return e;
  }
  if (int e = seg_loss_grad(logits_lo, reinterpret_cast<const long long*>(labels), n_valid_ws,
                            reinterpret_cast<long long*>(pred), dlogit_hi, loss, logits_hi, batch, h, w, H, W, 19, 255, S(stream)))
    return e;
  if (dlogit_lo) return logits_bilinear_bwd(dlogit_hi, BF(dlogit_lo), batch, h, w, H, W, 19, 32, 32, S(stream));
  return 0;
}
int wc_conv1_dgrad(const wc_bf16* dz, const float* weight, const float* scale, float* dx, int batch, int H, int W, void* stream) {
  return conv1_dgrad(BF(dz), weight, scale, dx, batch, H, W, 64, S(stream));
}
int wc_conv_in(const float* x, const float* weight, const float* bias, const float* scale, const float* shift,
               wc_bf16* y, int batch, int H, int W, int Cout, int K, int stride, int pad, int ldy, int relu,
               void* stream) {
  return conv_small_cin(x, weight, bias, scale, shift, BF(y), batch, 3, H, W, Cout, K, stride, pad, ldy, relu, S(stream));
}
int wc_conv_out(const wc_bf16* x, const float* weight, const float* bias, float* y, int batch, int H, int W, int Cin,
                int K, int ldx, int tanh_out, void* stream) {
  return conv_small_cout(BF(x), weight, bias, y, batch, H, W, Cin, 3, K, ldx, tanh_out, S(stream));
}
int wc_nchw_f32_to_nhwc_bf16(const float* x, wc_bf16* y, int batch, int C, int hw, int ldy, void* stream) {
  return nchw_f32_to_nhwc_bf16(x, BF(y), batch, C, hw, ldy, S(stream));
}
int wc_nhwc_bf16_to_nchw_f32(const wc_bf16* x, float* y, int batch, int C, int hw, int ldx, void* stream) {
  return nhwc_bf16_to_nchw_f32(BF(x), y, batch, C, hw, ldx, S(stream));
}
int wc_attention(const wc_bf16* q, const wc_bf16* k, const wc_bf16* vt, wc_bf16* out, int batch, int heads, int ntok,
                 int hd, int ldo, void* stream) {
  return attention_forward(BF(q), BF(k), BF(vt), BF(out), batch, heads, ntok, hd, ldo, S(stream));
}


int wc_attention_scaled(const wc_bf16* q, const wc_bf16* k, const wc_bf16* vt, wc_bf16* out, int batch, int heads, int ntok,
                        int hd, int ldo, float scale, void* stream) {
  return attention_forward(BF(q), BF(k), BF(vt), BF(out), batch, heads, ntok, hd, ldo, S(stream), nullptr, scale);
}

int wc_attention_lse(const wc_bf16* q, const wc_bf16* k, const wc_bf16* vt, wc_bf16* out, float* lse, int batch, int heads,
                     int ntok, int hd, int ldo, void* stream) {
  return attention_forward(BF(q), BF(k), BF(vt), BF(out), batch, heads, ntok, hd, ldo, S(stream), lse);
}

int wc_attention_bwd(const wc_bf16* q, const wc_bf16* k, const wc_bf16* v, const wc_bf16* o, const wc_bf16* d_o, const float* lse,
                     float* d_scratch, wc_bf16* dqkv, int batch, int heads, int ntok, int hd, void* stream) {
  const int C = heads * hd;
  if (int e = attn_rowdot(BF(o), BF(d_o), C, C, batch, ntok, heads, hd, d_scratch, S(stream))) return e;
  return attention_backward(BF(q), BF(k), BF(v), BF(d_o), C, lse, d_scratch, BF(dqkv), 3 * C, batch, heads, ntok, hd, S(stream));
}

int wc_conv2d_wgrad(const wc_bf16* x, const wc_bf16* dy, int batch, int H, int W, int Cin, int Cout, int K, int stride, int pad,
                    int dil, int transposed, const wc_bf16* x2, int Cin2, float* dw, float* dw2, void* stream) {
  cudaStream_t st = S(stream);
  DeviceArena arena;
  float* partial = static_cast<float*>(arena.alloc(kWgradPartialBytes));
  if (!partial) return 1;
  const int Ho = transposed ? H * 2 : H / stride, Wo = transposed ? W * 2 : W / stride;
  Act xa; xa.ptr = const_cast<__nv_bfloat16*>(BF(x)); xa.B = batch; xa.H = H; xa.W = W; xa.C = Cin; xa.ld = Cin;
  Act dya; dya.ptr = const_cast<__nv_bfloat16*>(BF(dy)); dya.B = batch; dya.H = Ho; dya.W = Wo; dya.C = Cout; dya.ld = Cout;
  Act x2a = xa; x2a.ptr = const_cast<__nv_bfloat16*>(BF(x2)); x2a.C = Cin2; x2a.ld = Cin2;
  WgradOp op;
  int e = transposed ? build_convT_wgrad(&op, xa, dya, K, pad, dw, partial)
                     : build_conv_wgrad(&op, xa, dya, K, stride, pad, dil, dw, x2 ? &x2a : nullptr, dw2, partial);
  if (e) return e;
  if ((e = op.run(st))) return e;
  WC_CHECK_CUDA(cudaStreamSynchronize(st));
  return 0;
}

size_t wc_groupnorm_bwd_workspace_bytes(int batch, int channels) { return groupnorm_bwd_workspace_bytes(batch, channels); }
int wc_groupnorm_silu_bwd(const wc_bf16* x, const wc_bf16* dy, wc_bf16* dx, int batch, int hw, int channels, const float* gamma,
                          const float* beta, float eps, int silu, const void* fwd_workspace, const wc_bf16* add1,
                          const wc_bf16* add2, float* dgamma, float* dbeta, void* workspace, void* stream) {
  return groupnorm_silu_bwd(BF(x), BF(dy), BF(dx), batch, hw, channels, channels, channels, channels, gamma, beta, eps, silu,
                            fwd_workspace, BF(add1), channels, BF(add2), channels, dgamma, dbeta, workspace, S(stream));
}
int wc_colsum(const wc_bf16* x, int batch, int hw, int channels, float* out_rows, float* out_total, void* workspace, void* stream) {
  return colsum(BF(x), batch, hw, channels, channels, out_rows, channels, out_total, workspace, S(stream));
}
int wc_mse_loss_grad(const float* pred, const float* target, float* dpred, size_t n, float grad_scale, float* loss, void* scratch,
                     void* stream) {
  return mse_loss_grad(pred, target, dpred, n, grad_scale, loss, scratch, S(stream));
}
size_t wc_boundary_wgrad_scratch_bytes(void) { return boundary_wgrad_scratch_bytes(); }
int wc_boundary_wgrad(const wc_bf16* wide, const float* narrow, int batch, int H, int W, int sign, float* dw, float* dbias,
                      void* scratch, void* stream) {
  return boundary_wgrad(BF(wide), 64, narrow, batch, H, W, sign, dw, dbias, scratch, S(stream));
}
int wc_adam_step(float* p, const float* g, float* m, float* v, size_t n, float lr, float beta1, float beta2, float eps, int step,
                 float grad_scale, void* stream) {
  return adam_step(p, g, m, v, n, lr, beta1, beta2, eps, step, grad_scale, S(stream));
}


int wc_ddpm_grid_u8(const float* x, uint8_t* out, int batch, int H, int W, int nrow, int padding, void* stream) {
  return ddpm_grid_u8(x, out, batch, H, W, nrow, padding, S(stream));
}
int wc_postprocess_u8(const float* x, uint8_t* out, int batch, int H, int W, const float* mean3_host, const float* std3_host, void* stream) {
  return postprocess_u8(x, out, batch, H, W, mean3_host, std3_host, S(stream));
}
int wc_label_encode(const uint8_t* label_ids, int Ws, const int* ytab, const int* xtab, int top, int left, int Hc, int Wc,
                    const int64_t* lut, int nlut, int64_t* out, void* stream) {
  return label_encode(label_ids, Ws, ytab, xtab, top, left, Hc, Wc, reinterpret_cast<const long long*>(lut), nlut,
                      reinterpret_cast<long long*>(out), S(stream));
}
int wc_resample_u8(const uint8_t* in, uint8_t* tmp, uint8_t* out, int Hin, int Win, int Hout, int Wout, int channels, const int* bounds_h,
                   const int* kk_h, int ksize_h, const int* bounds_v, const int* kk_v, int ksize_v, void* stream) {
  return resample_u8(in, tmp, out, Hin, Win, Hout, Wout, channels, bounds_h, kk_h, ksize_h, bounds_v, kk_v, ksize_v, S(stream));
}
int wc_u8_to_tensor(const uint8_t* in, int Win, int top, int left, int Hc, int Wc, int mode, const float* mean3_host, const float* std3_host,
                    float* out, void* stream) {
  return u8_to_tensor(in, Win, top, left, Hc, Wc, mode, mean3_host, std3_host, out, S(stream));
}

}
```

weatherconverter_b200/ops.py:

```python
import torch

from . import _lib
from ._lib import check, lib, ptr, require_cuda, stream_ptr


def to_nhwc_bf16(x: torch.Tensor) -> torch.Tensor:
    require_cuda(x)
    x = x.contiguous().float()
    B, Cc, H, W = x.shape
    y = torch.empty(B, H, W, Cc, device=x.device, dtype=torch.bfloat16)
    check(lib().wc_nchw_f32_to_nhwc_bf16(ptr(x), ptr(y), B, Cc, H * W, Cc, stream_ptr()))
    return y


def to_nchw_f32(x: torch.Tensor) -> torch.Tensor:
    require_cuda(x)
    B, H, W, Cc = x.shape
    assert x.stride(3) == 1 and x.stride(1) == W * x.stride(2) and x.stride(0) == H * x.stride(1)
    y = torch.empty(B, Cc, H, W, device=x.device, dtype=torch.float32)
    check(lib().wc_nhwc_bf16_to_nchw_f32(ptr(x), ptr(y), B, Cc, H * W, x.stride(2), stream_ptr()))
    return y


def groupnorm_silu(x, gamma, beta, silu=True, eps=1e-5):
    require_cuda(x, gamma, beta)
    B, H, W, Cc = x.shape
    y = torch.empty(B, H, W, Cc, device=x.device, dtype=torch.bfloat16)
    ws = torch.empty(lib().wc_groupnorm_workspace_bytes(B), device=x.device, dtype=torch.uint8)
    check(lib().wc_groupnorm_silu(ptr(x), ptr(y), B, H * W, Cc, x.stride(2), Cc, ptr(gamma), ptr(beta), eps,
                                  1 if silu else 0, ptr(ws), stream_ptr()))
    return y


def conv2d(x, weight, bias=None, stride=1, pad=None, dil=1, transposed=False, rowbias=None, residual=None,
           x2=None, weight2=None, relu=False):
    require_cuda(x, weight)
    B, H, W, Cin = x.shape
    K = weight.shape[-1]
    Cout = weight.shape[1] if transposed else weight.shape[0]
    if pad is None:
        pad = dil * (K - 1) // 2
    Ho, Wo = (2 * H, 2 * W) if transposed else ((H // 2, W // 2) if stride == 2 else (H, W))
    y = torch.empty(B, Ho, Wo, Cout, device=x.device, dtype=torch.bfloat16)
    weight = weight.contiguous().float()
    if weight2 is not None:
        weight2 = weight2.contiguous().float()
    check(lib().wc_conv2d(ptr(x), B, H, W, Cin, x.stride(2), ptr(weight), ptr(bias), Cout, K, stride, pad, dil,
                          1 if transposed else 0, ptr(rowbias), ptr(residual),
                          residual.stride(2) if residual is not None else 0,
                          ptr(x2), x2.shape[3] if x2 is not None else 0, x2.stride(2) if x2 is not None else 0,
                          ptr(weight2), 1 if relu else 0, ptr(y), Cout, stream_ptr()))
    return y


def conv_in(x, weight, bias=None, scale=None, shift=None, stride=1, pad=None, relu=False):
    require_cuda(x, weight)
    B, Cc, H, W = x.shape
    Cout, _, K, _ = weight.shape
    if pad is None:
        pad = K // 2
    Ho, Wo = (H + 2 * pad - K) // stride + 1, (W + 2 * pad - K) // stride + 1
    y = torch.empty(B, Ho, Wo, Cout, device=x.device, dtype=torch.bfloat16)
    x, weight = x.contiguous(), weight.contiguous()
    check(lib().wc_conv_in(ptr(x), ptr(weight), ptr(bias), ptr(scale), ptr(shift), ptr(y),
                           B, H, W, Cout, K, stride, pad, Cout, 1 if relu else 0, stream_ptr()))
    return y


def conv_out(x, weight, bias=None, tanh_out=False):
    require_cuda(x, weight)
    B, H, W, Cin = x.shape
    K = weight.shape[-1]
    y = torch.empty(B, 3, H, W, device=x.device, dtype=torch.float32)
    weight = weight.contiguous()
    check(lib().wc_conv_out(ptr(x), ptr(weight), ptr(bias), ptr(y), B, H, W, Cin, K, x.stride(2),
                            1 if tanh_out else 0, stream_ptr()))
    return y


def attention(q, k, vt, scale=0.0):
    require_cuda(q, k, vt)
    B, h, N, hd = q.shape
    out = torch.empty(B, N, h * hd, device=q.device, dtype=torch.bfloat16)
    q, k, vt = q.contiguous(), k.contiguous(), vt.contiguous()
    if scale == 0.0:
        check(lib().wc_attention(ptr(q), ptr(k), ptr(vt), ptr(out), B, h, N, hd, h * hd, stream_ptr()))
    else:
        check(lib().wc_attention_scaled(ptr(q), ptr(k), ptr(vt), ptr(out), B, h, N, hd, h * hd, float(scale), stream_ptr()))
    return out


def ddpm_step(xt, eps, z, beta, sqrt_one_minus_acp, sqrt_alpha, sigma, want_parts=False):
    require_cuda(xt, eps, z)
    xt, eps = xt.contiguous(), eps.contiguous()
    B = xt.shape[0]
    n = xt[0].numel()
    out = torch.empty_like(xt)
    mean = torch.empty_like(xt) if want_parts else None
    sigz = torch.empty_like(xt) if (want_parts and z is not None) else None
    z = z.contiguous() if z is not None else None
    check(lib().wc_ddpm_step(ptr(xt), ptr(eps), ptr(z), ptr(out), ptr(mean),
                             ptr(sigz), n, B, float(beta), float(sqrt_one_minus_acp), float(sqrt_alpha), float(sigma),
                             stream_ptr()))
    return (out, mean, sigz) if want_parts else out


def launch_count() -> int:
    return int(lib().wc_launch_count())


def attention_lse(q, k, vt):
    require_cuda(q, k, vt)
    B, h, N, hd = q.shape
    out = torch.empty(B, N, h * hd, device=q.device, dtype=torch.bfloat16)
    lse = torch.empty(B * h, N, device=q.device, dtype=torch.float32)
    q, k, vt = q.contiguous(), k.contiguous(), vt.contiguous()
    check(lib().wc_attention_lse(ptr(q), ptr(k), ptr(vt), ptr(out), ptr(lse), B, h, N, hd, h * hd, stream_ptr()))
    return out, lse


def attention_bwd(q, k, v, o, d_o, lse):
    require_cuda(q, k, v, o, d_o, lse)
    B, h, N, hd = q.shape
    q, k, v, o, d_o = q.contiguous(), k.contiguous(), v.contiguous(), o.contiguous(), d_o.contiguous()
    dqkv = torch.zeros(B, N, 3 * h * hd, device=q.device, dtype=torch.bfloat16)
    scratch = torch.empty(B * h * N, device=q.device, dtype=torch.float32)
    check(lib().wc_attention_bwd(ptr(q), ptr(k), ptr(v), ptr(o), ptr(d_o), ptr(lse), ptr(scratch), ptr(dqkv), B, h, N, hd,
                                 stream_ptr()))
    return dqkv


def conv2d_wgrad(x, dy, K, stride=1, pad=None, dil=1, transposed=False, x2=None):
    require_cuda(x, dy)
    B, H, W, Cin = x.shape
    Cout = dy.shape[3]
    if pad is None:
        pad = dil * (K - 1) // 2
    x, dy = x.contiguous(), dy.contiguous()
    shape = (Cin, Cout, K, K) if transposed else (Cout, Cin, K, K)
    dw = torch.full(shape, float("nan"), device=x.device, dtype=torch.float32)
    dw2 = None
    if x2 is not None:
        x2 = x2.contiguous()
        dw2 = torch.full((Cout, x2.shape[3], 1, 1), float("nan"), device=x.device, dtype=torch.float32)
    check(lib().wc_conv2d_wgrad(ptr(x), ptr(dy), B, H, W, Cin, Cout, K, stride, pad, dil, 1 if transposed else 0,
                                ptr(x2), x2.shape[3] if x2 is not None else 0, ptr(dw), ptr(dw2), stream_ptr()))
    return (dw, dw2) if x2 is not None else dw


def groupnorm_silu_fwd_bwd(x, gamma, beta, dy, silu=True, eps=1e-5, add1=None, add2=None):
    require_cuda(x, gamma, beta, dy)
    B, H, W, Cc = x.shape
    x, dy = x.contiguous(), dy.contiguous()
    y = torch.empty_like(x)
    ws = torch.empty(lib().wc_groupnorm_workspace_bytes(B), device=x.device, dtype=torch.uint8)
    check(lib().wc_groupnorm_silu(ptr(x), ptr(y), B, H * W, Cc, Cc, Cc, ptr(gamma), ptr(beta), eps, 1 if silu else 0,
                                  ptr(ws), stream_ptr()))
    dx = torch.empty_like(x)
    dg = torch.empty(Cc, device=x.device, dtype=torch.float32)
    db = torch.empty(Cc, device=x.device, dtype=torch.float32)
    ws2 = torch.empty(lib().wc_groupnorm_bwd_workspace_bytes(B, Cc), device=x.device, dtype=torch.uint8)
    add1 = add1.contiguous() if add1 is not None else None
    add2 = add2.contiguous() if add2 is not None else None
    check(lib().wc_groupnorm_silu_bwd(ptr(x), ptr(dy), ptr(dx), B, H * W, Cc, ptr(gamma), ptr(beta), eps, 1 if silu else 0,
                                      ptr(ws), ptr(add1), ptr(add2), ptr(dg), ptr(db), ptr(ws2), stream_ptr()))
    return y, dx, dg, db


def colsum(x):
    require_cuda(x)
    B, H, W, Cc = x.shape
    x = x.contiguous()
    rows = torch.empty(B, Cc, device=x.device, dtype=torch.float32)
    tot = torch.empty(Cc, device=x.device, dtype=torch.float32)
    ws = torch.empty(lib().wc_groupnorm_bwd_workspace_bytes(B, Cc), device=x.device, dtype=torch.uint8)
    check(lib().wc_colsum(ptr(x), B, H * W, Cc, ptr(rows), ptr(tot), ptr(ws), stream_ptr()))
    return rows, tot


def mse_loss_grad(pred, target, grad_scale=1.0):
    require_cuda(pred, target)
    pred, target = pred.contiguous(), target.contiguous()
    dpred = torch.empty_like(pred)
    loss = torch.empty(1, device=pred.device, dtype=torch.float32)
    scratch = torch.empty(8192, device=pred.device, dtype=torch.uint8)
    check(lib().wc_mse_loss_grad(ptr(pred), ptr(target), ptr(dpred), pred.numel(), float(grad_scale), ptr(loss), ptr(scratch),
                                 stream_ptr()))
    return loss, dpred


def boundary_wgrad(wide, narrow, sign):
    require_cuda(wide, narrow)
    B, H, W, Cc = wide.shape
    assert Cc == 64
    wide, narrow = wide.contiguous(), narrow.contiguous()
    dw = torch.empty((64, 3, 3, 3) if sign > 0 else (3, 64, 3, 3), device=wide.device, dtype=torch.float32)
    db = torch.empty(64 if sign > 0 else 3, device=wide.device, dtype=torch.float32)
    scratch = torch.empty(lib().wc_boundary_wgrad_scratch_bytes(), device=wide.device, dtype=torch.uint8)
    check(lib().wc_boundary_wgrad(ptr(wide), ptr(narrow), B, H, W, sign, ptr(dw), ptr(db), ptr(scratch), stream_ptr()))
    return dw, db


def adam_step(p, g, m, v, lr, beta1, beta2, eps, step, grad_scale=1.0):
    require_cuda(p, g, m, v)
    check(lib().wc_adam_step(ptr(p), ptr(g), ptr(m), ptr(v), p.numel(), lr, beta1, beta2, eps, step, grad_scale, stream_ptr()))
```

Before: 3.005.

## Add five-softmax-group variant of small-head attention kernel, default for hd16

Templates the small-head tcgen05 attention kernel on the number of 128-row query groups per CTA and adds a 5-group variant. It trims service and softmax register budgets, reduces K stages or P buffers to fit shared memory, and for hd32 splits TMEM score loads into halves to save registers. The 5-group path becomes the default for head_dim 16, with poly 12, and an API is exposed to select groups explicitly. The aim is more query rows per CTA to amortise K/V loads and keep the tensor core busier, at the cost of tighter registers and shallower pipelining.

```diff
diff --git a/include/wc_b200.h b/include/wc_b200.h
--- a/include/wc_b200.h
+++ b/include/wc_b200.h
@@ -87,6 +87,8 @@
 
 int wc_attention_lse(const wc_bf16* q, const wc_bf16* k, const wc_bf16* vt, wc_bf16* out, float* lse, int batch, int heads,
                      int ntok, int hd, int ldo, void* stream);
+int wc_attention_small_groups(const wc_bf16* q, const wc_bf16* k, const wc_bf16* vt, wc_bf16* out, float* lse, int batch,
+                              int heads, int ntok, int hd, int ldo, float scale, int groups, int poly, void* stream);
 int wc_attention_bwd(const wc_bf16* q, const wc_bf16* k, const wc_bf16* v, const wc_bf16* o, const wc_bf16* d_o, const float* lse,
                      float* d_scratch, wc_bf16* dqkv, int batch, int heads, int ntok, int hd, void* stream);
 int wc_conv2d_wgrad(const wc_bf16* x, const wc_bf16* dy, int batch, int H, int W, int Cin, int Cout, int K, int stride, int pad,
diff --git a/weatherconverter_b200/_lib.py b/weatherconverter_b200/_lib.py
--- a/weatherconverter_b200/_lib.py
+++ b/weatherconverter_b200/_lib.py
@@ -66,6 +66,7 @@
     "wc_attention_lse": (C.c_int, [c_ptr] * 5 + [C.c_int] * 5 + [c_ptr]),
     "wc_attention_scaled": (C.c_int, [c_ptr] * 4 + [C.c_int] * 5 + [C.c_float, c_ptr]),
     "wc_attention_bwd": (C.c_int, [c_ptr] * 8 + [C.c_int] * 4 + [c_ptr]),
+    "wc_attention_small_groups": (C.c_int, [c_ptr] * 5 + [C.c_int] * 5 + [C.c_float, C.c_int, C.c_int, c_ptr]),
     "wc_conv2d_wgrad": (C.c_int, [c_ptr, c_ptr] + [C.c_int] * 10 + [c_ptr, C.c_int, c_ptr, c_ptr, c_ptr]),
     "wc_groupnorm_bwd_workspace_bytes": (C.c_size_t, [C.c_int, C.c_int]),
     "wc_groupnorm_silu_bwd": (C.c_int, [c_ptr] * 3 + [C.c_int] * 3 + [c_ptr, c_ptr, C.c_float, C.c_int] + [c_ptr] * 7),
diff --git a/weatherconverter_b200/csrc/attention.cu b/weatherconverter_b200/csrc/attention.cu
--- a/weatherconverter_b200/csrc/attention.cu
+++ b/weatherconverter_b200/csrc/attention.cu
@@ -391,7 +391,8 @@
 int attention_small_forward(const __nv_bfloat16* q, const __nv_bfloat16* k, const __nv_bfloat16* vt, __nv_bfloat16* out, int B,
                             int heads, int ntok, int hd, int ldo, cudaStream_t st, float* lse, float scale);
 int attention_small4_forward(const __nv_bfloat16* q, const __nv_bfloat16* k, const __nv_bfloat16* vt, __nv_bfloat16* out, int B,
-                             int heads, int ntok, int hd, int ldo, cudaStream_t st, float* lse, float scale);
+                             int heads, int ntok, int hd, int ldo, cudaStream_t st, float* lse, float scale, int groups,
+                             int poly);
 
 int attention_forward(const __nv_bfloat16* q, const __nv_bfloat16* k, const __nv_bfloat16* vt, __nv_bfloat16* out, int B,
                       int heads, int ntok, int hd, int ldo, cudaStream_t st, float* lse, float scale) {
@@ -413,7 +414,7 @@
       const char* e = getenv("WC_ATTN_SMALL4_HD32");
       four32 = e ? atoi(e) : 1;
     }
-    if (four && (hd == 16 || (hd == 32 && four32)) && ntok >= 2048) return attention_small4_forward(q, k, vt, out, B, heads, ntok, hd, ldo, st, lse, scale);
+    if (four && (hd == 16 || (hd == 32 && four32)) && ntok >= 2048) return attention_small4_forward(q, k, vt, out, B, heads, ntok, hd, ldo, st, lse, scale, 0, 0);
     return attention_small_forward(q, k, vt, out, B, heads, ntok, hd, ldo, st, lse, scale);
   }
   static int tp = -1;
diff --git a/weatherconverter_b200/csrc/attention_small4.cu b/weatherconverter_b200/csrc/attention_small4.cu
--- a/weatherconverter_b200/csrc/attention_small4.cu
+++ b/weatherconverter_b200/csrc/attention_small4.cu
@@ -21,20 +21,16 @@
 };
 
 constexpr int kBKV = 64;
-constexpr int kNQ = 4;
-constexpr int kKStages = 4;
 constexpr float kShift = 8.0f;
 constexpr float kLazy = 6.0f;
-#ifndef WC_S4_SERVICE_REGS
-#define WC_S4_SERVICE_REGS 56
-#define WC_S4_SOFTMAX_REGS 104
-#endif
-constexpr int kRegsService = WC_S4_SERVICE_REGS, kRegsSoftmax = WC_S4_SOFTMAX_REGS;
-static_assert(128 * kRegsService + 512 * kRegsSoftmax <= 640 * 96, "register pool of the CTA");
-
-template <int HD>
+
+template <int HD, int NQ>
 struct Cfg4 {
-  static constexpr bool kLT = true;
+  static_assert(NQ == 4 || NQ == 5, "four or five softmax groups");
+  static constexpr bool kLT = !(HD == 32 && NQ == 5);
+  static constexpr bool kSplitS = NQ == 5;
+  static constexpr int kKStages = (HD == 16 && NQ == 5) ? 3 : 4;
+  static constexpr int kPBufs = (HD == 32 && NQ == 5) ? 1 : 2;
   static constexpr int kRowBytes = HD * 2;
   static constexpr int kSwz = HD * 2;
   static constexpr int kKSteps = HD / 16;
@@ -46,11 +42,20 @@
   static constexpr uint32_t kVBlock = kVRows * 128;
   static constexpr uint32_t kVLoad = HD * 128;
   static constexpr uint32_t kPTile = 128 * kBKV * 2;
-  static constexpr uint32_t kSmem = kNQ * kQTile + kNQ * kXTile + kKxTile + kKStages * (kKTile + kVBlock) + 2 * kNQ * kPTile + 1024 + 512;
-  static constexpr int kThreads = 128 + 128 * kNQ;
+  static constexpr uint32_t kSmem = NQ * kQTile + NQ * kXTile + kKxTile + kKStages * (kKTile + kVBlock) + kPBufs * NQ * kPTile + 1024 + 512;
+  static_assert(kSmem <= 227 * 1024, "shared memory budget");
+  static constexpr int kThreads = 128 + 128 * NQ;
   static constexpr int kColsPerQ = kBKV + kVRows;
-  static_assert(kNQ * kColsPerQ <= 512, "TMEM budget");
+  static_assert(NQ * kColsPerQ <= 512, "TMEM budget");
   static constexpr uint32_t kTmemCols = 512;
+  static constexpr int kRegsLaunch = NQ == 4 ? 96 : 80;
+  static constexpr int kRegsService = NQ == 4 ? 56 : 40;
+  static constexpr int kRegsSoftmax = NQ == 4 ? 104 : 88;
+  static_assert(kThreads * kRegsLaunch <= 65536, "launch allocation");
+  static_assert(128 * kRegsService + 128 * NQ * kRegsSoftmax <= kThreads * kRegsLaunch, "register pool of the CTA");
+  static constexpr int kBarK = 1, kBarKE = 5, kBarV = 9, kBarVE = 13, kBarSF = 17, kBarSR = kBarSF + NQ, kBarPF = kBarSR + NQ,
+                       kBarPD = kBarPF + 2 * NQ, kBarQR = kBarPD + 2 * NQ, kBarSlot = kBarQR + NQ;
+  static_assert(kKStages <= 4 && 8 * kBarSlot + 4 <= 512, "barrier slots");
 };
 
 __device__ __forceinline__ void sts128(uint32_t addr, uint32_t a, uint32_t b, uint32_t c, uint32_t d) {
@@ -88,38 +93,40 @@
   return o;
 }
 
-template <int HD, int POLY, bool UNIT>
-__global__ void __launch_bounds__(Cfg4<HD>::kThreads, 1)
+template <int HD, int POLY, bool UNIT, int NQ>
+__global__ void __launch_bounds__(Cfg4<HD, NQ>::kThreads, 1)
 attention_small4_kernel(const __grid_constant__ Small4Maps maps, const __grid_constant__ Small4Args p) {
-  using Cfg = Cfg4<HD>;
+  using Cfg = Cfg4<HD, NQ>;
   constexpr bool LT = Cfg::kLT;
+  constexpr int kKStages = Cfg::kKStages, NB = Cfg::kPBufs;
+  constexpr bool SPLIT = Cfg::kSplitS;
   extern __shared__ uint8_t smem_raw[];
   const uint32_t base = (smem_u32(smem_raw) + 1023u) & ~1023u;
   const uint32_t q_smem = base;
-  const uint32_t qx_smem = q_smem + kNQ * Cfg::kQTile;
-  const uint32_t kx_smem = qx_smem + kNQ * Cfg::kXTile;
+  const uint32_t qx_smem = q_smem + NQ * Cfg::kQTile;
+  const uint32_t kx_smem = qx_smem + NQ * Cfg::kXTile;
   const uint32_t k_smem = kx_smem + Cfg::kKxTile;
   const uint32_t v_smem = k_smem + kKStages * Cfg::kKTile;
   const uint32_t p_smem = v_smem + kKStages * Cfg::kVBlock;
-  const uint32_t bars = p_smem + 2 * kNQ * Cfg::kPTile;
+  const uint32_t bars = p_smem + NB * NQ * Cfg::kPTile;
   const uint32_t q_full = bars;
-  auto k_full = [&](int s) { return bars + 8u * (1 + s); };
-  auto k_empty = [&](int s) { return bars + 8u * (5 + s); };
-  auto v_full = [&](int s) { return bars + 8u * (9 + s); };
-  auto v_empty = [&](int s) { return bars + 8u * (13 + s); };
-  auto s_full = [&](int q) { return bars + 8u * (17 + q); };
-  auto s_free = [&](int q) { return bars + 8u * (21 + q); };
-  auto p_full = [&](int q, int b) { return bars + 8u * (25 + 2 * q + b); };
-  auto pv_done = [&](int q, int b) { return bars + 8u * (33 + 2 * q + b); };
-  auto q_ready = [&](int q) { return bars + 8u * (41 + q); };
-  const uint32_t tmem_slot = bars + 8u * 45;
+  auto k_full = [&](int s) { return bars + 8u * (Cfg::kBarK + s); };
+  auto k_empty = [&](int s) { return bars + 8u * (Cfg::kBarKE + s); };
+  auto v_full = [&](int s) { return bars + 8u * (Cfg::kBarV + s); };
+  auto v_empty = [&](int s) { return bars + 8u * (Cfg::kBarVE + s); };
+  auto s_full = [&](int q) { return bars + 8u * (Cfg::kBarSF + q); };
+  auto s_free = [&](int q) { return bars + 8u * (Cfg::kBarSR + q); };
+  auto p_full = [&](int q, int b) { return bars + 8u * (Cfg::kBarPF + 2 * q + b); };
+  auto pv_done = [&](int q, int b) { return bars + 8u * (Cfg::kBarPD + 2 * q + b); };
+  auto q_ready = [&](int q) { return bars + 8u * (Cfg::kBarQR + q); };
+  const uint32_t tmem_slot = bars + 8u * Cfg::kBarSlot;
   volatile uint32_t* tmem_slot_ptr = reinterpret_cast<volatile uint32_t*>(smem_raw + (tmem_slot - smem_u32(smem_raw)));
 
   const int warp = __shfl_sync(0xffffffffu, threadIdx.x >> 5, 0), lane = threadIdx.x & 31;
   const int bh = HD == 16 ? blockIdx.x : blockIdx.y;
-  const int q0 = (HD == 16 ? blockIdx.y : blockIdx.x) * (128 * kNQ);
+  const int q0 = (HD == 16 ? blockIdx.y : blockIdx.x) * (128 * NQ);
   const int nkv = (p.ntok + kBKV - 1) / kBKV;
-  const int nq_valid = min(kNQ, (p.ntok - q0 + 127) / 128);
+  const int nq_valid = min(NQ, (p.ntok - q0 + 127) / 128);
 
   if (warp == 0 && lane == 0) {
     tma_prefetch_desc(&maps.q);
@@ -132,10 +139,10 @@
       mbar_init(k_full(s), 1); mbar_init(k_empty(s), 1);
       mbar_init(v_full(s), 1); mbar_init(v_empty(s), 1);
     }
-    for (int q = 0; q < kNQ; ++q) {
+    for (int q = 0; q < NQ; ++q) {
       mbar_init(s_full(q), 1);
       mbar_init(s_free(q), 128);
-      for (int b = 0; b < 2; ++b) {
+      for (int b = 0; b < NB; ++b) {
         mbar_init(p_full(q, b), 128);
         mbar_init(pv_done(q, b), 1);
       }
@@ -155,11 +162,11 @@
   const uint32_t tmem_base = *tmem_slot_ptr;
 
   if (warp < 4) {
-    asm volatile("setmaxnreg.dec.sync.aligned.u32 %0;" ::"n"(kRegsService));
+    asm volatile("setmaxnreg.dec.sync.aligned.u32 %0;" ::"n"(Cfg::kRegsService));
     if (warp == 0) {
       if (lane == 0) {
-        mbar_arrive_expect_tx(q_full, kNQ * Cfg::kQTile);
-        for (int q = 0; q < kNQ; ++q) tma_load_3d(q_smem + q * Cfg::kQTile, &maps.q, q_full, 0, q0 + q * 128, bh);
+        mbar_arrive_expect_tx(q_full, NQ * Cfg::kQTile);
+        for (int q = 0; q < NQ; ++q) tma_load_3d(q_smem + q * Cfg::kQTile, &maps.q, q_full, 0, q0 + q * 128, bh);
         for (int j = 0; j < nkv; ++j) {
           const int s = j % kKStages;
           const uint32_t ph = (j / kKStages) & 1u;
@@ -190,7 +197,7 @@
       };
       mbar_wait(k_full(0), 0);
 #pragma unroll
-      for (int q = 0; q < kNQ; ++q) {
+      for (int q = 0; q < NQ; ++q) {
         mbar_wait(q_ready(q), 0);
         tc_fence_after();
         if (q < nq_valid) {
@@ -204,7 +211,7 @@
         const int s1 = (j + 1) % kKStages;
         mbar_wait(k_full(s1), ((j + 1) / kKStages) & 1u);
 #pragma unroll
-        for (int q = 0; q < kNQ; ++q) {
+        for (int q = 0; q < NQ; ++q) {
           if (q < nq_valid) {
             mbar_wait(s_free(q), j & 1u);
             tc_fence_after();
@@ -225,17 +232,17 @@
         const int s = j % kKStages;
         mbar_wait(v_full(s), (j / kKStages) & 1u);
 #pragma unroll
-        for (int q = 0; q < kNQ; ++q) {
+        for (int q = 0; q < NQ; ++q) {
           if (q < nq_valid) {
-            mbar_wait(p_full(q, j & 1), (j >> 1) & 1u);
+            mbar_wait(p_full(q, j % NB), (j / NB) & 1u);
             tc_fence_after();
             if (elect_one_sync()) {
               const uint32_t d = tmem_u + q * Cfg::kColsPerQ + kBKV;
-              const uint32_t p_lo = p_lo0 + (2 * q + (j & 1)) * (Cfg::kPTile >> 4), v_lo = v_lo0 + s * (Cfg::kVBlock >> 4);
+              const uint32_t p_lo = p_lo0 + (NB * q + j % NB) * (Cfg::kPTile >> 4), v_lo = v_lo0 + s * (Cfg::kVBlock >> 4);
 #pragma unroll
               for (int k = 0; k < 4; ++k)
                 umma_bf16(d, umma_desc_join(p_lo + 2u * k, hi_pv), umma_desc_join(v_lo + 2u * k, hi_pv), idesc_o, (j | k) != 0 ? 1u : 0u);
-              umma_commit(pv_done(q, j & 1));
+              umma_commit(pv_done(q, j % NB));
             }
             __syncwarp();
           }
@@ -245,14 +252,14 @@
       }
     }
   } else {
-    asm volatile("setmaxnreg.inc.sync.aligned.u32 %0;" ::"n"(kRegsSoftmax));
+    asm volatile("setmaxnreg.inc.sync.aligned.u32 %0;" ::"n"(Cfg::kRegsSoftmax));
     const int q = (warp - 4) >> 2;
     const int quad = warp & 3;
     const int row = quad * 32 + lane;
     const uint32_t lane_off = static_cast<uint32_t>(quad * 32) << 16;
     const uint32_t s_tmem = tmem_base + q * Cfg::kColsPerQ + lane_off;
     const uint32_t o_tmem = s_tmem + kBKV;
-    const uint32_t p_row = p_smem + 2 * q * Cfg::kPTile + row * 128;
+    const uint32_t p_row = p_smem + NB * q * Cfg::kPTile + row * 128;
     const uint32_t qx_row = qx_smem + q * Cfg::kXTile + row * 32;
 
     const float cs = p.c;
@@ -266,7 +273,7 @@
       }
       if (LT) {
         constexpr int kChunks = kKStages * 16 * 8;
-        for (int c = t; c < kChunks; c += 128 * kNQ) {
+        for (int c = t; c < kChunks; c += 128 * NQ) {
           const int blk = c >> 7, r = (c >> 3) & 15, ch = c & 7;
           const uint32_t one = r == 0 ? 0x3F803F80u : 0u;
           sts128(v_smem + blk * Cfg::kVBlock + (HD + r) * 128 + ch * 16, one, one, one, one);
@@ -296,17 +303,27 @@
     float carry = 0.f;
 
     for (int j = 0; j < (q < nq_valid ? nkv : 0); ++j) {
-      const int b = j & 1;
+      const int b = j % NB;
       const int kv0 = j * kBKV;
       mbar_wait(s_full(q), j & 1u);
-      if (j >= 2) mbar_wait(pv_done(q, b), ((j - 2) >> 1) & 1u);
+      if (j >= NB) mbar_wait(pv_done(q, b), ((j - NB) / NB) & 1u);
       tc_fence_after();
       uint32_t ra[32], rb[32], w[16];
-      tmem_ld32(s_tmem, ra);
-      tmem_ld32(s_tmem + 32, rb);
-      tmem_wait_ld();
-      tc_fence_before();
-      mbar_arrive(s_free(q));
+      uint32_t (&rh)[32] = SPLIT ? ra : rb;
+      auto load_half = [&](int c) {
+        if (SPLIT) {
+          tmem_ld32(s_tmem + 32 * c, ra);
+          tmem_wait_ld();
+        }
+      };
+      if (!SPLIT) {
+        tmem_ld32(s_tmem, ra);
+        tmem_ld32(s_tmem + 32, rb);
+        tmem_wait_ld();
+        tc_fence_before();
+        mbar_arrive(s_free(q));
+      }
+      bool upd = false;
       const bool tail = (kv0 + kBKV > p.ntok);
       bool slow = tail || j == 0 || __any_sync(0xffffffffu, carry != 0.f);
       const uint32_t blk = p_row + b * Cfg::kPTile;
@@ -340,8 +357,10 @@
             sts128(blk + (static_cast<uint32_t>(chunk ^ (row & 7)) << 4), w[4 * ch], w[4 * ch + 1], w[4 * ch + 2], w[4 * ch + 3]);
           }
         };
+        load_half(0);
         half(ra, 0);
-        half(rb, 1);
+        load_half(1);
+        half(rh, 1);
         bool redo;
         if (LT) {
           redo = (orw & 0xC000C000u) != 0u;
@@ -354,25 +373,38 @@
       }
       if (slow) {
         float tmax = -INFINITY;
-#pragma unroll
-        for (int i = 0; i < 32; ++i) {
-          float a0 = __uint_as_float(ra[i]), a1 = __uint_as_float(rb[i]);
-          if (tail && kv0 + i >= p.ntok) a0 = -INFINITY;
-          if (tail && kv0 + 32 + i >= p.ntok) a1 = -INFINITY;
-          tmax = fmaxf(tmax, fmaxf(a0, a1));
+        if (SPLIT) {
+#pragma unroll
+          for (int c = 0; c < 2; ++c) {
+            load_half(c);
+#pragma unroll
+            for (int i = 0; i < 32; ++i) {
+              float a = __uint_as_float(ra[i]);
+              if (tail && kv0 + 32 * c + i >= p.ntok) a = -INFINITY;
+              tmax = fmaxf(tmax, a);
+            }
+          }
+        } else {
+#pragma unroll
+          for (int i = 0; i < 32; ++i) {
+            float a0 = __uint_as_float(ra[i]), a1 = __uint_as_float(rb[i]);
+            if (tail && kv0 + i >= p.ntok) a0 = -INFINITY;
+            if (tail && kv0 + 32 + i >= p.ntok) a1 = -INFINITY;
+            tmax = fmaxf(tmax, fmaxf(a0, a1));
+          }
         }
         tmax -= carry;
         float delta = 0.f;
-        const bool upd = (j == 0) || (tmax > -shift + kLazy / cs);
+        upd = (j == 0) || (tmax > -shift + kLazy / cs);
         if (upd) {
-          if (j + 1 < nkv) mbar_wait(s_full(q), (j + 1) & 1u);
+          if (!SPLIT && j + 1 < nkv) mbar_wait(s_full(q), (j + 1) & 1u);
           const float e_new = bf16_round(E + tmax + shift);
           delta = e_new - E;
           E = e_new;
-          sts16(qx_row, bf16_bits(-e_new));
+          if (!SPLIT) sts16(qx_row, bf16_bits(-e_new));
         }
         if (j > 0 && __any_sync(0xffffffffu, upd)) {
-          mbar_wait(pv_done(q, (j - 1) & 1), ((j - 1) >> 1) & 1u);
+          mbar_wait(pv_done(q, (j - 1) % NB), ((j - 1) / NB) & 1u);
           tc_fence_after();
           const float alpha = ex2_approx(-delta * cs);
           if (!LT) {
@@ -410,15 +442,25 @@
             sts128(blk + (static_cast<uint32_t>(chunk ^ (row & 7)) << 4), w[4 * ch], w[4 * ch + 1], w[4 * ch + 2], w[4 * ch + 3]);
           }
         };
+        load_half(0);
         redo_half(ra, 0, lsum[0]);
-        redo_half(rb, 1, lsum[1]);
+        load_half(1);
+        redo_half(rh, 1, lsum[1]);
+      }
+      if (SPLIT) {
+        tc_fence_before();
+        mbar_arrive(s_free(q));
+        if (upd) {
+          if (j + 1 < nkv) mbar_wait(s_full(q), (j + 1) & 1u);
+          sts16(qx_row, bf16_bits(-E));
+        }
       }
       fence_proxy_async_smem();
       tc_fence_before();
       mbar_arrive(p_full(q, b));
     }
 
-    if (q < nq_valid) mbar_wait(pv_done(q, (nkv - 1) & 1), ((nkv - 1) >> 1) & 1u);
+    if (q < nq_valid) mbar_wait(pv_done(q, (nkv - 1) % NB), ((nkv - 1) / NB) & 1u);
     tc_fence_after();
     const int tok = q0 + q * 128 + row;
     const int bb = bh / p.heads, head = bh % p.heads;
@@ -455,10 +497,10 @@
   }
 }
 
-template <int HD, int POLY, bool UNIT>
+template <int HD, int POLY, bool UNIT, int NQ>
 int launch_small4_p(const __nv_bfloat16* q, const __nv_bfloat16* k, const __nv_bfloat16* vt, __nv_bfloat16* out, int B, int heads,
                     int ntok, int ldo, cudaStream_t st, float* lse, float scale) {
-  using Cfg = Cfg4<HD>;
+  using Cfg = Cfg4<HD, NQ>;
   Small4Maps maps;
   const int BH = B * heads;
   {
@@ -486,50 +528,70 @@
   }
   static bool attr_set = false;
   if (!attr_set) {
-    WC_CHECK_CUDA(cudaFuncSetAttribute(attention_small4_kernel<HD, POLY, UNIT>, cudaFuncAttributeMaxDynamicSharedMemorySize, Cfg::kSmem));
+    WC_CHECK_CUDA(cudaFuncSetAttribute(attention_small4_kernel<HD, POLY, UNIT, NQ>, cudaFuncAttributeMaxDynamicSharedMemorySize, Cfg::kSmem));
     attr_set = true;
   }
-  const int nqb = (ntok + 128 * kNQ - 1) / (128 * kNQ);
+  const int nqb = (ntok + 128 * NQ - 1) / (128 * NQ);
   dim3 grid(HD == 16 ? BH : nqb, HD == 16 ? nqb : BH);
   ProfScope prof(kProfAttention, st, 4.0 * BH * static_cast<double>(ntok) * ntok * HD);
   prof.note(BH, ntok, HD);
-  launch_k<1>(attention_small4_kernel<HD, POLY, UNIT>, grid, Cfg::kThreads, Cfg::kSmem, st, maps, args);
+  launch_k<1>(attention_small4_kernel<HD, POLY, UNIT, NQ>, grid, Cfg::kThreads, Cfg::kSmem, st, maps, args);
   WC_LAUNCH_CHECK();
   return 0;
 }
 
-template <int HD>
+template <int HD, int NQ>
 int launch_small4(const __nv_bfloat16* q, const __nv_bfloat16* k, const __nv_bfloat16* vt, __nv_bfloat16* out, int B, int heads,
-                  int ntok, int ldo, cudaStream_t st, float* lse, float scale) {
-  static int poly = -1;
-  if (poly < 0) {
+                  int ntok, int ldo, cudaStream_t st, float* lse, float scale, int poly_arg) {
+  static int poly_env = -1;
+  if (poly_env < 0) {
     const char* e = getenv("WC_ATTN_SMALL4_POLY");
-    poly = e ? atoi(e) : 8;
-  }
+    poly_env = e ? atoi(e) : (NQ == 5 ? 12 : 8);
+  }
+  const int poly = poly_arg ? poly_arg : poly_env;
   const bool unit = attn_scale_log2(scale, HD) == 1.f;
   {
     if (unit) {
       switch (poly) {
-        case 8: return launch_small4_p<HD, 8, true>(q, k, vt, out, B, heads, ntok, ldo, st, lse, scale);
-        case 16: return launch_small4_p<HD, 16, true>(q, k, vt, out, B, heads, ntok, ldo, st, lse, scale);
-        default: return launch_small4_p<HD, 12, true>(q, k, vt, out, B, heads, ntok, ldo, st, lse, scale);
+        case 8: return launch_small4_p<HD, 8, true, NQ>(q, k, vt, out, B, heads, ntok, ldo, st, lse, scale);
+        case 16: return launch_small4_p<HD, 16, true, NQ>(q, k, vt, out, B, heads, ntok, ldo, st, lse, scale);
+        default: return launch_small4_p<HD, 12, true, NQ>(q, k, vt, out, B, heads, ntok, ldo, st, lse, scale);
       }
     }
   }
   switch (poly) {
-    case 8: return launch_small4_p<HD, 8, false>(q, k, vt, out, B, heads, ntok, ldo, st, lse, scale);
-    case 16: return launch_small4_p<HD, 16, false>(q, k, vt, out, B, heads, ntok, ldo, st, lse, scale);
-    default: return launch_small4_p<HD, 12, false>(q, k, vt, out, B, heads, ntok, ldo, st, lse, scale);
+    case 8: return launch_small4_p<HD, 8, false, NQ>(q, k, vt, out, B, heads, ntok, ldo, st, lse, scale);
+    case 16: return launch_small4_p<HD, 16, false, NQ>(q, k, vt, out, B, heads, ntok, ldo, st, lse, scale);
+    default: return launch_small4_p<HD, 12, false, NQ>(q, k, vt, out, B, heads, ntok, ldo, st, lse, scale);
   }
 }
 
 }
 
 int attention_small4_forward(const __nv_bfloat16* q, const __nv_bfloat16* k, const __nv_bfloat16* vt, __nv_bfloat16* out, int B,
-                             int heads, int ntok, int hd, int ldo, cudaStream_t st, float* lse, float scale) {
-  switch (hd) {
-    case 16: return launch_small4<16>(q, k, vt, out, B, heads, ntok, ldo, st, lse, scale);
-    case 32: return launch_small4<32>(q, k, vt, out, B, heads, ntok, ldo, st, lse, scale);
+                             int heads, int ntok, int hd, int ldo, cudaStream_t st, float* lse, float scale, int groups,
+                             int poly) {
+  static int five16 = -1, five32 = -1;
+  if (five16 < 0) {
+    const char* e = getenv("WC_ATTN_SMALL5");
+    const char* v = e ? e : "16";
+    five16 = five32 = 0;
+    while (*v) {
+      char* end = nullptr;
+      const long d = strtol(v, &end, 10);
+      if (end == v) break;
+      five16 |= d == 16;
+      five32 |= d == 32;
+      v = *end == ',' ? end + 1 : end;
+    }
+  }
+  if (groups == 0) groups = (hd == 16 ? five16 : hd == 32 ? five32 : 0) ? 5 : 4;
+  if (groups != 4 && groups != 5) return fail("attention_small4: groups must be 4 or 5, got " + std::to_string(groups));
+  switch (hd * 10 + groups) {
+    case 164: return launch_small4<16, 4>(q, k, vt, out, B, heads, ntok, ldo, st, lse, scale, poly);
+    case 165: return launch_small4<16, 5>(q, k, vt, out, B, heads, ntok, ldo, st, lse, scale, poly);
+    case 324: return launch_small4<32, 4>(q, k, vt, out, B, heads, ntok, ldo, st, lse, scale, poly);
+    case 325: return launch_small4<32, 5>(q, k, vt, out, B, heads, ntok, ldo, st, lse, scale, poly);
     default: return fail("attention_small4: unsupported head_dim " + std::to_string(hd));
   }
 }
diff --git a/weatherconverter_b200/csrc/wc_api.cu b/weatherconverter_b200/csrc/wc_api.cu
--- a/weatherconverter_b200/csrc/wc_api.cu
+++ b/weatherconverter_b200/csrc/wc_api.cu
@@ -37,6 +37,9 @@
 int prof_stop(double* ms, long long* count, double* work);
 int attention_forward(const __nv_bfloat16* q, const __nv_bfloat16* k, const __nv_bfloat16* vt, __nv_bfloat16* out, int B,
                       int heads, int ntok, int hd, int ldo, cudaStream_t st, float* lse = nullptr, float scale = 0.f);
+int attention_small4_forward(const __nv_bfloat16* q, const __nv_bfloat16* k, const __nv_bfloat16* vt, __nv_bfloat16* out, int B,
+                             int heads, int ntok, int hd, int ldo, cudaStream_t st, float* lse, float scale, int groups,
+                             int poly);
 int maxpool_fwd(const __nv_bfloat16* x, __nv_bfloat16* y, uint8_t* idx, int B, int H, int W, int C, cudaStream_t st);
 int maxpool_bwd(const __nv_bfloat16* dy, const uint8_t* idx, const __nv_bfloat16* x, __nv_bfloat16* dx, int B, int H,
                 int W, int C, cudaStream_t st);
@@ -276,6 +279,15 @@
   return attention_forward(BF(q), BF(k), BF(vt), BF(out), batch, heads, ntok, hd, ldo, S(stream), lse);
 }
 
+int wc_attention_small_groups(const wc_bf16* q, const wc_bf16* k, const wc_bf16* vt, wc_bf16* out, float* lse, int batch,
+                              int heads, int ntok, int hd, int ldo, float scale, int groups, int poly, void* stream) {
+  WC_REQUIRE(hd == 16 || hd == 32, "head_dim must be 16 or 32");
+  WC_REQUIRE(ntok % 8 == 0, "token count must be a multiple of 8");
+  WC_REQUIRE(ldo % 8 == 0, "output row stride must be a multiple of 8");
+  WC_REQUIRE(poly == 0 || poly == 8 || poly == 12 || poly == 16, "poly must be 0, 8, 12 or 16");
+  return attention_small4_forward(BF(q), BF(k), BF(vt), BF(out), batch, heads, ntok, hd, ldo, S(stream), lse, scale, groups, poly);
+}
+
 int wc_attention_bwd(const wc_bf16* q, const wc_bf16* k, const wc_bf16* v, const wc_bf16* o, const wc_bf16* d_o, const float* lse,
                      float* d_scratch, wc_bf16* dqkv, int batch, int heads, int ntok, int hd, void* stream) {
   const int C = heads * hd;
diff --git a/weatherconverter_b200/ops.py b/weatherconverter_b200/ops.py
--- a/weatherconverter_b200/ops.py
+++ b/weatherconverter_b200/ops.py
@@ -119,6 +119,17 @@
     return out, lse
 
 
+def attention_small_groups(q, k, vt, groups, scale=0.0, poly=0):
+    require_cuda(q, k, vt)
+    B, h, N, hd = q.shape
+    out = torch.empty(B, N, h * hd, device=q.device, dtype=torch.bfloat16)
+    lse = torch.empty(B * h, N, device=q.device, dtype=torch.float32)
+    q, k, vt = q.contiguous(), k.contiguous(), vt.contiguous()
+    check(lib().wc_attention_small_groups(ptr(q), ptr(k), ptr(vt), ptr(out), ptr(lse), B, h, N, hd, h * hd, float(scale),
+                                          int(groups), int(poly), stream_ptr()))
+    return out, lse
+
+
 def attention_bwd(q, k, v, o, d_o, lse):
     require_cuda(q, k, v, o, d_o, lse)
     B, h, N, hd = q.shape
```

Result: no change. 3.034 (median of 6 runs) (+1.0%).
